# delehef/asgart

Measured on AMD Instinct MI355X. Metric: Mbp/s probe+extend (direct+RC, k=20 g=100), higher is better.
Workload: dtype u64 keys / u32 SA

## Files before the change

asgart_amd/__init__.py:

```python
from __future__ import annotations

import ctypes as C
import os
from dataclasses import dataclass, field
from typing import List, Optional, Sequence, Tuple

import numpy as np

__all__ = [
    "AsgartError", "RunSettings", "ProtoSD", "Strand", "Index", "Searcher", "SearchDuplications",
    "load_library", "library_path", "ABI_SYMBOLS", "sa_build64", "search_duplications_multi", "merge_shards",
    "score_owners", "score_costs", "compute_scores_multi", "Source", "compute_scores_flags_multi", "orientation_flags",
]

_HERE = os.path.dirname(os.path.abspath(__file__))

ABI_SYMBOLS = (
    "asgart_sa_build64", "asgart_index_create", "asgart_index_destroy", "asgart_index_prepare",
    "asgart_search_duplications", "asgart_search_duplications_shard", "asgart_families_counts",
    "asgart_families_copy", "asgart_families_free", "asgart_searcher_cache_get",
    "asgart_searcher_search", "asgart_sa_read", "asgart_probe_hits", "asgart_get_stats",
    "asgart_last_error", "asgart_version", "asgart_compute_scores", "asgart_index_set_option",
    "asgart_index_check_sa", "asgart_index_create_trim", "asgart_index_clone",
    "asgart_search_duplications_multi", "asgart_search_duplications_ex", "asgart_search_duplications_passes",
    "asgart_search_duplications_passes_shard", "asgart_families_keys",
    "asgart_index_export", "asgart_index_create_device", "asgart_trim_cache", "asgart_post_process",
    "asgart_debug_dump_stacks", "asgart_prepare_data", "asgart_score_owners", "asgart_score_costs",
    "asgart_compute_scores_shard", "asgart_compute_scores_multi", "asgart_tier_plan",
    "asgart_source_create", "asgart_source_destroy", "asgart_extract_sequences",
    "asgart_compute_scores_flags", "asgart_compute_scores_flags_shard", "asgart_compute_scores_flags_multi",
    "asgart_fasta_read", "asgart_fasta_counts", "asgart_fasta_copy", "asgart_fasta_read_text", "asgart_fasta_index",
    "asgart_fasta_source", "asgart_fasta_free", "asgart_fasta_timings", "asgart_fasta_geometry",
)


def merge_shards(parts) -> Tuple[np.ndarray, np.ndarray]:
    keys = np.concatenate([p[2] for p in parts]) if parts else np.zeros(0, np.uint64)
    if len(keys) == 0:
        return np.zeros(1, np.uint64), np.zeros((0, 4), np.uint64)
    starts = np.concatenate([p[0][:-1].astype(np.int64) + b for p, b in
                             zip(parts, np.cumsum([0] + [len(p[1]) for p in parts[:-1]]))])
    lens = np.concatenate([np.diff(p[0].astype(np.int64)) for p in parts])
    sds = np.concatenate([p[1] for p in parts])
    order = np.argsort(keys, kind="stable")
    lens_o, starts_o = lens[order], starts[order]
    offs = np.concatenate([[0], np.cumsum(lens_o)]).astype(np.uint64)
    idx = np.repeat(starts_o - offs[:-1].astype(np.int64), lens_o) + np.arange(int(offs[-1]), dtype=np.int64)
    return offs, sds[idx]


class AsgartError(RuntimeError):
    def __init__(self, code: int, msg: str):
        super().__init__(f"libasgart_hip error {code}: {msg}")
        self.code = code


def library_path() -> str:
    return os.environ.get("ASGART_LIB") or os.path.join(_HERE, "libasgart_hip.so")


class _Settings(C.Structure):
    _fields_ = [
        ("probe_size", C.c_uint64),
        ("max_gap_size", C.c_uint32),
        ("min_duplication_length", C.c_uint64),
        ("max_cardinality", C.c_uint64),
        ("reverse", C.c_uint8),
        ("complement", C.c_uint8),
    ]


class Stats(C.Structure):
    _fields_ = [("ms_total", C.c_double), ("ms_search", C.c_double), ("ms_scan", C.c_double),
                ("ms_fill", C.c_double), ("ms_extend", C.c_double)] + [
        (n, C.c_uint64) for n in (
            "probes_total", "probes_n_skipped", "probes_searched", "probes_card_skipped",
            "probes_with_hits", "raw_hits", "filtered_hits", "segments", "families", "proto_sds",
            "bisect_steps", "search_launches", "overflow_segments")] + [("ms_extend_tier2", C.c_double), ("heavy_segments", C.c_uint64), ("ms_probe_count", C.c_double),
        ("search_bytes", C.c_uint64), ("probes_filter_rejected", C.c_uint64), ("search_bytes_wide_loads", C.c_uint64),
        ("ms_longest_tier", C.c_double), ("passes", C.c_uint64), ("ms_longest_segment", C.c_double),
        ("split_segments", C.c_uint64), ("split_refused", C.c_uint64)]

    def as_dict(self):
        return {n: getattr(self, n) for n, _ in self._fields_}


_lib: Optional[C.CDLL] = None


def load_library() -> C.CDLL:
    global _lib
    if _lib is not None:
        return _lib
    path = library_path()
    if not os.path.exists(path):
        raise AsgartError(-3, f"{path} not built: run `python -c 'import __graft_entry__ as g; "
                              f"g.build()'` (hipcc --offload-arch=gfx950); there is no CPU fallback")
    L = C.CDLL(path)
    vp, u64p = C.c_void_p, C.POINTER(C.c_uint64)
    L.asgart_sa_build64.argtypes = [vp, vp, C.c_int64]
    L.asgart_sa_build64.restype = C.c_int32
    L.asgart_index_create.argtypes = [vp, C.c_int64, vp, C.c_int64, C.c_int32, C.POINTER(vp)]
    L.asgart_index_create.restype = C.c_int32
    L.asgart_index_create_trim.argtypes = [vp, C.c_int64, vp, C.c_int64, C.c_int64, C.c_int64, C.c_int32,
                                           C.POINTER(vp)]
    L.asgart_index_create_trim.restype = C.c_int32
    L.asgart_index_clone.argtypes = [vp, C.c_int32, C.POINTER(vp)]
    L.asgart_index_clone.restype = C.c_int32
    L.asgart_index_export.argtypes = [vp, C.POINTER(vp), C.POINTER(vp), C.POINTER(C.c_int32)]
    L.asgart_index_export.restype = C.c_int32
    L.asgart_index_create_device.argtypes = [vp, C.c_int64, vp, C.c_int64, C.c_int32, C.c_int32, C.POINTER(vp)]
    L.asgart_index_create_device.restype = C.c_int32
    L.asgart_trim_cache.argtypes = [C.c_int32]
    L.asgart_trim_cache.restype = C.c_int64
    L.asgart_prepare_data.argtypes = [vp, vp, C.c_int64, C.c_int32, C.c_int32, vp, vp, C.c_int64, C.POINTER(C.c_int64),
# ... 8 lines not shown
    L.asgart_fasta_read.argtypes = [vp, vp, C.c_int64, C.c_int32, C.c_int32, C.POINTER(vp)]
    L.asgart_fasta_read.restype = C.c_int32
    L.asgart_fasta_counts.argtypes = [vp, C.POINTER(C.c_int64), C.POINTER(C.c_int64), u64p]
    L.asgart_fasta_counts.restype = C.c_int32
    L.asgart_fasta_copy.argtypes = [vp, vp, vp, vp]
    L.asgart_fasta_copy.restype = C.c_int32
    L.asgart_fasta_read_text.argtypes = [vp, C.c_uint64, C.c_uint64, vp]
    L.asgart_fasta_read_text.restype = C.c_int32
    L.asgart_fasta_index.argtypes = [vp, C.POINTER(vp)]
    L.asgart_fasta_index.restype = C.c_int32
    L.asgart_fasta_source.argtypes = [vp, C.POINTER(vp)]
    L.asgart_fasta_source.restype = C.c_int32
    L.asgart_fasta_free.argtypes = [vp]
    L.asgart_fasta_free.restype = None
    L.asgart_fasta_timings.argtypes = [vp, C.POINTER(C.c_double)]
    L.asgart_fasta_timings.restype = C.c_int32
    L.asgart_fasta_geometry.argtypes = [u64p, u64p, u64p]
    L.asgart_fasta_geometry.restype = None
    L.asgart_debug_dump_stacks.argtypes = []
    L.asgart_debug_dump_stacks.restype = C.c_int32
    L.asgart_post_process.argtypes = [vp, vp, C.c_uint64, vp, C.c_int32, C.POINTER(vp)]
    L.asgart_post_process.restype = C.c_int32
    L.asgart_search_duplications_multi.argtypes = [C.POINTER(vp), C.c_int32, vp, C.c_int64, C.POINTER(_Settings), vp,
                                                   C.POINTER(vp)]
    L.asgart_search_duplications_multi.restype = C.c_int32
    L.asgart_index_destroy.argtypes = [vp]
    L.asgart_index_destroy.restype = None
    L.asgart_index_set_option.argtypes = [vp, C.c_char_p, C.c_int64]
    L.asgart_index_set_option.restype = C.c_int32
    L.asgart_index_check_sa.argtypes = [vp]
    L.asgart_index_check_sa.restype = C.c_int64
    L.asgart_index_prepare.argtypes = [vp, C.c_uint64]
    L.asgart_index_prepare.restype = C.c_int32
    L.asgart_search_duplications.argtypes = [vp, vp, C.c_int64, C.POINTER(_Settings), vp,
                                             C.POINTER(vp)]
    L.asgart_search_duplications.restype = C.c_int32
    L.asgart_search_duplications_shard.argtypes = [vp, vp, C.c_int64, C.POINTER(_Settings),
                                                   C.c_int32, C.c_int32, C.POINTER(vp)]
    L.asgart_search_duplications_shard.restype = C.c_int32
    L.asgart_search_duplications_ex.argtypes = [vp, vp, C.c_int64, C.POINTER(_Settings), C.c_int32, C.c_int32, vp,
                                                C.POINTER(vp)]
    L.asgart_search_duplications_ex.restype = C.c_int32
    L.asgart_search_duplications_passes.argtypes = [vp, vp, C.c_int64, C.POINTER(_Settings), C.c_int32, C.POINTER(vp)]
    L.asgart_search_duplications_passes.restype = C.c_int32
    L.asgart_families_keys.argtypes = [vp, vp]
    L.asgart_families_keys.restype = None
    L.asgart_search_duplications_passes_shard.argtypes = [vp, vp, C.c_int64, C.POINTER(_Settings), C.c_int32, C.c_int32,
                                                          C.c_int32, C.POINTER(vp)]
    L.asgart_search_duplications_passes_shard.restype = C.c_int32
    L.asgart_families_counts.argtypes = [vp, u64p, u64p]
    L.asgart_families_counts.restype = None
    L.asgart_families_copy.argtypes = [vp, vp, vp]
    L.asgart_families_copy.restype = None
    L.asgart_families_free.argtypes = [vp]
    L.asgart_families_free.restype = None
    L.asgart_searcher_cache_get.argtypes = [vp, vp, C.c_int64, vp, vp]
    L.asgart_searcher_cache_get.restype = C.c_int32
    L.asgart_searcher_search.argtypes = [vp, vp, C.c_int64, C.c_uint64, vp, vp]
    L.asgart_searcher_search.restype = C.c_int32
    L.asgart_sa_read.argtypes = [vp, C.c_uint64, C.c_uint64, vp]
    L.asgart_sa_read.restype = C.c_int32
    L.asgart_compute_scores.argtypes = [vp, vp, C.c_int64, C.c_int32, C.c_int32, vp]
    L.asgart_compute_scores.restype = C.c_int32
    L.asgart_score_owners.argtypes = [vp, C.c_int64, C.c_int32, vp]
    L.asgart_score_owners.restype = C.c_int32
    L.asgart_score_costs.argtypes = [vp, C.c_int64, vp]
    L.asgart_score_costs.restype = C.c_int32
    L.asgart_tier_plan.argtypes = [C.c_int32, vp, C.c_int64, vp, C.c_double, vp, vp]
    L.asgart_tier_plan.restype = C.c_int32
    L.asgart_compute_scores_shard.argtypes = [vp, vp, C.c_int64, C.c_int32, C.c_int32, C.c_int32, C.c_int32, vp]
    L.asgart_compute_scores_shard.restype = C.c_int64
    L.asgart_compute_scores_multi.argtypes = [C.POINTER(vp), C.c_int32, vp, C.c_int64, C.c_int32, C.c_int32, vp]
    L.asgart_compute_scores_multi.restype = C.c_int32
    L.asgart_compute_scores_flags.argtypes = [vp, vp, vp, C.c_int64, vp]
    L.asgart_compute_scores_flags.restype = C.c_int32
    L.asgart_compute_scores_flags_shard.argtypes = [vp, vp, vp, C.c_int64, C.c_int32, C.c_int32, vp]
    L.asgart_compute_scores_flags_shard.restype = C.c_int64
    L.asgart_compute_scores_flags_multi.argtypes = [C.POINTER(vp), C.c_int32, vp, vp, C.c_int64, vp]
    L.asgart_compute_scores_flags_multi.restype = C.c_int32
    L.asgart_probe_hits.argtypes = [vp, vp, C.c_int64, C.POINTER(_Settings), vp, vp, vp, u64p]
    L.asgart_probe_hits.restype = C.c_int64
    L.asgart_get_stats.argtypes = [vp, C.c_uint32, C.POINTER(Stats)]
    L.asgart_get_stats.restype = C.c_int32
    L.asgart_last_error.argtypes = []
    L.asgart_last_error.restype = C.c_char_p
    L.asgart_version.argtypes = []
    L.asgart_version.restype = C.c_char_p
    _lib = L
    return L


def _check(rc: int):
    if rc < 0:
        raise AsgartError(int(rc), load_library().asgart_last_error().decode(errors="replace"))


def _ptr(a: Optional[np.ndarray]):
    return None if a is None else a.ctypes.data_as(C.c_void_p)


def _as_u8(seq) -> np.ndarray:
    if isinstance(seq, np.ndarray):
        if seq.dtype != np.uint8:
            raise TypeError("text must be uint8")
        return np.ascontiguousarray(seq)
    if isinstance(seq, str):
        seq = seq.encode()
    return np.frombuffer(bytes(seq), dtype=np.uint8).copy()


@dataclass
class RunSettings:

    probe_size: int = 20
    max_gap_size: int = 120
    min_duplication_length: int = 1000
    max_cardinality: int = 500
    reverse: bool = False
    complement: bool = False
    skip_masked: bool = False
    trim: Optional[Tuple[int, int]] = None

    @classmethod
    def from_cli(cls, k=20, gap=100, min_length=1000, max_cardinality=500, reverse=False,
                 complement=False, skip_masked=False) -> "RunSettings":
        return cls(k, gap + k, min_length, max_cardinality, reverse, complement, skip_masked)

    def _c(self) -> _Settings:
        return _Settings(self.probe_size, self.max_gap_size, self.min_duplication_length,
                         self.max_cardinality, int(self.reverse), int(self.complement))


@dataclass
class ProtoSD:

    left: int
    right: int
    left_length: int
    right_length: int
    identity: float = 0.0
    reversed: bool = False
    complemented: bool = False

    def as_tuple(self):
        return (self.left, self.right, self.left_length, self.right_length)


ProtoSDsFamily = List[ProtoSD]


@dataclass
class Strand:

    file_names: str
    data: np.ndarray
    map: list = field(default_factory=list)


class Index:

    def __init__(self, text, sa: Optional[np.ndarray] = None, device: int = 0,
                 trim: Optional[Tuple[int, int]] = None):
        L = load_library()
        self.text = _as_u8(text)
        self.n = len(self.text)
        self._h = C.c_void_p()
        self.trim = trim
        sa_arr = None
        want = len(self.text) if trim is None else trim[1] - trim[0] + 1
        if sa is not None:
            sa_arr = np.ascontiguousarray(sa, dtype=np.int64)
            if len(sa_arr) != want:
                raise ValueError("suffix array length != text length (or the trimmed window + 1)")
        if trim is None:
            _check(L.asgart_index_create(_ptr(self.text), len(self.text), _ptr(sa_arr),
                                         want if sa_arr is not None else 0, device, C.byref(self._h)))
        else:
            _check(L.asgart_index_create_trim(_ptr(self.text), len(self.text), _ptr(sa_arr),
                                              want if sa_arr is not None else 0, int(trim[0]), int(trim[1]),
                                              device, C.byref(self._h)))

    def close(self):
        if getattr(self, "_h", None) and self._h.value:
            load_library().asgart_index_destroy(self._h)
            self._h = C.c_void_p()

    def __del__(self):
        try:
            self.close()
        except Exception:
            pass

    def __enter__(self):
        return self

    def __exit__(self, *exc):
        self.close()

    def clone(self, device: int = 0) -> "Index":
        other = Index.__new__(Index)
        other.text = self.text
        other.n = self.n
        other.trim = self.trim
        other._h = C.c_void_p()
        _check(load_library().asgart_index_clone(self._h, device, C.byref(other._h)))
        return other

    def export(self) -> Tuple[int, int, int]:
        t, a, w = C.c_void_p(), C.c_void_p(), C.c_int32()
        _check(load_library().asgart_index_export(self._h, C.byref(t), C.byref(a), C.byref(w)))
        return int(t.value), int(a.value), int(w.value)

    @classmethod
    def from_device(cls, d_text: int, n: int, d_sa: int, sa_entry_bytes: int, device: int = 0, text=None) -> "Index":
        self = cls.__new__(cls)
        self.text = text
        self.n = int(n)
        self.trim = None
        self._h = C.c_void_p()
        _check(load_library().asgart_index_create_device(C.c_void_p(d_text), n, C.c_void_p(d_sa), n, sa_entry_bytes,
                                                         device, C.byref(self._h)))
        return self

    def set_option(self, name: str, value: int):
        _check(load_library().asgart_index_set_option(self._h, name.encode(), int(value)))

    def check_sa(self) -> int:
        r = int(load_library().asgart_index_check_sa(self._h))
        _check(r)
        return r

    def prepare(self, probe_size: int):
        _check(load_library().asgart_index_prepare(self._h, probe_size))

    def sa_read(self, lo: int, hi: int) -> np.ndarray:
        out = np.empty(max(0, hi - lo), dtype=np.int64)
        _check(load_library().asgart_sa_read(self._h, lo, hi, _ptr(out)))
        return out

    def compute_scores(self, sds: np.ndarray, reversed_: bool = False, complemented: bool = False) -> np.ndarray:
        sds = np.ascontiguousarray(sds, dtype=np.uint64).reshape(-1, 4)
        out = np.empty(len(sds), dtype=np.float32)
        _check(load_library().asgart_compute_scores(self._h, _ptr(sds), len(sds), int(reversed_),
                                                    int(complemented), _ptr(out)))
        return out

    def compute_scores_shard(self, sds: np.ndarray, reversed_: bool = False, complemented: bool = False,
                             shard: int = 0, n_shards: int = 1) -> np.ndarray:
        sds = np.ascontiguousarray(sds, dtype=np.uint64).reshape(-1, 4)
        out = np.full(len(sds), np.nan, dtype=np.float32)
        _check(load_library().asgart_compute_scores_shard(self._h, _ptr(sds), len(sds), int(reversed_),
                                                          int(complemented), int(shard), int(n_shards), _ptr(out)))
        return out

    def compute_scores_flags(self, sds: np.ndarray, flags: Optional[np.ndarray]) -> np.ndarray:
        sds = np.ascontiguousarray(sds, dtype=np.uint64).reshape(-1, 4)
        flags = _score_flags(flags, len(sds))
        out = np.empty(len(sds), dtype=np.float32)
        _check(load_library().asgart_compute_scores_flags(self._h, _ptr(sds), _ptr(flags), len(sds), _ptr(out)))
        return out

    def compute_scores_flags_shard(self, sds: np.ndarray, flags: Optional[np.ndarray], shard: int = 0,
                                   n_shards: int = 1) -> np.ndarray:
        sds = np.ascontiguousarray(sds, dtype=np.uint64).reshape(-1, 4)
        flags = _score_flags(flags, len(sds))
        out = np.full(len(sds), np.nan, dtype=np.float32)
        _check(load_library().asgart_compute_scores_flags_shard(self._h, _ptr(sds), _ptr(flags), len(sds), int(shard),
                                                                int(n_shards), _ptr(out)))
        return out

    def post_process(self, offs: np.ndarray, sds: np.ndarray, threads: int = 0) -> Tuple[np.ndarray, np.ndarray]:
        L = load_library()
        offs = np.ascontiguousarray(offs, dtype=np.uint64)
        sds = np.ascontiguousarray(sds, dtype=np.uint64).reshape(-1, 4)
        h = C.c_void_p()
        _check(L.asgart_post_process(self._h, _ptr(offs), len(offs) - 1, _ptr(sds), threads, C.byref(h)))
        try:
            nf, ns = C.c_uint64(), C.c_uint64()
            L.asgart_families_counts(h, C.byref(nf), C.byref(ns))
            o = np.zeros(nf.value + 1, dtype=np.uint64)
            d = np.zeros((ns.value, 4), dtype=np.uint64)
            L.asgart_families_copy(h, _ptr(o), _ptr(d))
        finally:
            L.asgart_families_free(h)
        return o, d

    def stats(self, flags: int = 2) -> Stats:
        st = Stats()
        _check(load_library().asgart_get_stats(self._h, flags, C.byref(st)))
        return st

    def search_duplications_raw(self, chunks: Sequence[Tuple[int, int]], settings: RunSettings,
                                shard: int = 0, n_shards: int = 1, progress: Optional[np.ndarray] = None,
                                with_keys: bool = False):
        L = load_library()
        ch = np.array(chunks, dtype=np.uint64).reshape(-1)
        st = settings._c()
        h = C.c_void_p()
        if progress is not None:
            assert progress.dtype == np.uint64 and len(progress) >= len(chunks)
        if n_shards == 1:
            _check(L.asgart_search_duplications(self._h, _ptr(ch), len(chunks), C.byref(st), _ptr(progress),
                                                C.byref(h)))
        elif progress is None:
            _check(L.asgart_search_duplications_shard(self._h, _ptr(ch), len(chunks), C.byref(st),
                                                      shard, n_shards, C.byref(h)))
        else:
            _check(L.asgart_search_duplications_ex(self._h, _ptr(ch), len(chunks), C.byref(st), shard, n_shards,
# ... 94 lines not shown
        ends = np.zeros(2 * max(len(sds) - first, 1), dtype=np.uint64)
        done = C.c_int64()
        rc = load_library().asgart_extract_sequences(self._h, _ptr(sds), _ptr(flags), len(sds), int(first), _ptr(out),
                                                     len(out), _ptr(ends), C.byref(done))
        try:
            _check(rc)
        except AsgartError as err:
            if rc == -4:
                err.room = int(ends[1])
            raise
        return ends[:2 * done.value], int(done.value)

    def extract(self, sds: np.ndarray, reversed_=False, complemented=False,
                piece_bytes: int = 1 << 30) -> Tuple[np.ndarray, np.ndarray]:
        sds = np.ascontiguousarray(sds, dtype=np.uint64).reshape(-1, 4)
        n = len(sds)
        flags = (np.broadcast_to(np.asarray(reversed_, dtype=bool), (n,)).astype(np.uint8) |
                 (np.broadcast_to(np.asarray(complemented, dtype=bool), (n,)).astype(np.uint8) << 1))
        flags = np.ascontiguousarray(flags)
        total = int(sds[:, 2].sum(dtype=np.uint64) + sds[:, 3].sum(dtype=np.uint64)) if n else 0
        data = np.empty(total, dtype=np.uint8)
        ends = np.zeros(2 * n, dtype=np.uint64)
        first = pos = 0
        while first < n:
            cap = min(max(int(piece_bytes), 1), total - pos)
            try:
                e, done = self.extract_piece(sds, flags, first, data[pos:pos + cap])
            except AsgartError as err:
                if err.code != -4:
                    raise
                e, done = self.extract_piece(sds, flags, first, data[pos:pos + err.room])
            if done == 0:
                raise AsgartError(-4, f"asgart_extract_sequences: no progress at duplication {first}")
            ends[2 * first:2 * (first + done)] = e + np.uint64(pos)
            pos += int(e[-1]) if done else 0
            first += done
        return ends, data


def search_duplications_multi(indices: Sequence[Index], chunks: Sequence[Tuple[int, int]],
                              settings: RunSettings) -> Tuple[np.ndarray, np.ndarray]:
    L = load_library()
    ch = np.array(chunks, dtype=np.uint64).reshape(-1)
    st = settings._c()
    arr = (C.c_void_p * len(indices))(*[i._h for i in indices])
    h = C.c_void_p()
    _check(L.asgart_search_duplications_multi(arr, len(indices), _ptr(ch), len(chunks), C.byref(st), None,
                                              C.byref(h)))
    try:
        nf, ns = C.c_uint64(), C.c_uint64()
        L.asgart_families_counts(h, C.byref(nf), C.byref(ns))
        offs = np.zeros(nf.value + 1, dtype=np.uint64)
        sds = np.zeros((ns.value, 4), dtype=np.uint64)
        L.asgart_families_copy(h, _ptr(offs), _ptr(sds))
    finally:
        L.asgart_families_free(h)
    return offs, sds


def score_owners(sds: np.ndarray, n_shards: int) -> np.ndarray:
    sds = np.ascontiguousarray(sds, dtype=np.uint64).reshape(-1, 4)
    out = np.zeros(len(sds), dtype=np.int32)
    _check(load_library().asgart_score_owners(_ptr(sds), len(sds), int(n_shards), _ptr(out)))
    return out


def score_costs(sds: np.ndarray) -> np.ndarray:
    sds = np.ascontiguousarray(sds, dtype=np.uint64).reshape(-1, 4)
    out = np.zeros(len(sds), dtype=np.uint64)
    _check(load_library().asgart_score_costs(_ptr(sds), len(sds), _ptr(out)))
    return out


def tier_plan(budget: int, n_work, tier_order: int, est_ms, main_ms: float = 0.0) -> Tuple[np.ndarray, np.ndarray]:
    work = np.ascontiguousarray(n_work, dtype=np.uint64).reshape(7)
    est = np.ascontiguousarray(est_ms, dtype=np.float64).reshape(7)
    stream_of = np.zeros(7, dtype=np.int32)
    launch = np.zeros(7, dtype=np.int32)
    _check(load_library().asgart_tier_plan(int(budget), _ptr(work), int(tier_order), _ptr(est), float(main_ms),
                                           _ptr(stream_of), _ptr(launch)))
    return stream_of, launch


def compute_scores_multi(indices: Sequence[Index], sds: np.ndarray, reversed_: bool = False,
                         complemented: bool = False) -> np.ndarray:
    L = load_library()
    sds = np.ascontiguousarray(sds, dtype=np.uint64).reshape(-1, 4)
    out = np.empty(len(sds), dtype=np.float32)
    arr = (C.c_void_p * len(indices))(*[i._h for i in indices])
    _check(L.asgart_compute_scores_multi(arr, len(indices), _ptr(sds), len(sds), int(reversed_), int(complemented),
                                         _ptr(out)))
    return out


def _score_flags(flags, n: int) -> Optional[np.ndarray]:
    if flags is None:
        return None
    flags = np.ascontiguousarray(flags, dtype=np.uint8).reshape(-1)
    if len(flags) != n:
        raise ValueError(f"{len(flags)} flag bytes for {n} duplications")
    return flags


def orientation_flags(reversed_, complemented, n: Optional[int] = None) -> np.ndarray:
    f = np.asarray(reversed_, dtype=bool).astype(np.uint8) | (np.asarray(complemented, dtype=bool).astype(np.uint8) << 1)
    return np.ascontiguousarray(np.broadcast_to(f, (n,)) if n is not None else f)


def compute_scores_flags_multi(indices: Sequence[Index], sds: np.ndarray, flags: Optional[np.ndarray]) -> np.ndarray:
    sds = np.ascontiguousarray(sds, dtype=np.uint64).reshape(-1, 4)
    flags = _score_flags(flags, len(sds))
    out = np.empty(len(sds), dtype=np.float32)
    arr = (C.c_void_p * len(indices))(*[i._h for i in indices])
    _check(load_library().asgart_compute_scores_flags_multi(arr, len(indices), _ptr(sds), _ptr(flags), len(sds),
                                                            _ptr(out)))
    return out


def trim_cache(device: int = 0) -> int:
    r = int(load_library().asgart_trim_cache(device))
    _check(r)
    return r


def sa_build64(text) -> np.ndarray:
    t = _as_u8(text)
    sa = np.empty(len(t), dtype=np.int64)
    _check(load_library().asgart_sa_build64(_ptr(t), _ptr(sa), len(t)))
    return sa


class Searcher:

    def __init__(self, index: Index, offset: int = 0):
        self.index = index
        self.offset = offset

    @classmethod
    def new(cls, dna, sa: np.ndarray, offset: int = 0, device: int = 0) -> "Searcher":
        return cls(Index(dna, sa, device), offset)

    def cache(self, patterns8: Sequence[bytes]) -> List[Tuple[int, int]]:
        pats = np.frombuffer(b"".join(bytes(p) for p in patterns8), dtype=np.uint8).copy()
        n = len(patterns8)
        lo = np.zeros(n, dtype=np.uint64)
        hi = np.zeros(n, dtype=np.uint64)
        _check(load_library().asgart_searcher_cache_get(self.index._h, _ptr(pats), n, _ptr(lo),
                                                        _ptr(hi)))
        return [(int(a), int(b)) for a, b in zip(lo, hi)]

    def search_ranges(self, patterns: Sequence[bytes]) -> List[Tuple[int, int]]:
        k = len(patterns[0])
        pats = np.frombuffer(b"".join(bytes(p) for p in patterns), dtype=np.uint8).copy()
        n = len(patterns)
        lo = np.zeros(n, dtype=np.uint64)
        hi = np.zeros(n, dtype=np.uint64)
        _check(load_library().asgart_searcher_search(self.index._h, _ptr(pats), n, k, _ptr(lo),
                                                     _ptr(hi)))
        return [(int(a), int(b)) for a, b in zip(lo, hi)]

    def search(self, pattern: bytes) -> List[Tuple[int, int]]:
        (lo, hi), = self.search_ranges([pattern])
        starts = self.index.sa_read(lo, hi)
        k = len(pattern)
        return [(self.offset + int(x), self.offset + int(x) + k) for x in starts]

# ... 31 lines not shown
```

asgart_amd/csrc/device_base.hpp:

```cpp
#pragma once

#include "search_dev.hpp"

#include <type_traits>

namespace asgart {

constexpr int kTiers = 7;
constexpr int kRunsStat = kTiers + 1;

enum Counter {
    CT_BIG = 0,
    CT_SEG,
    CT_SCAN_TICKET,
    CT_FAM,
    CT_SD,
    CT_OVF,
    CT_TOTAL_HITS,
    CT_N_SKIPPED,
    CT_CARD_SKIPPED,
    CT_WITH_HITS,
    CT_RAW_HITS,
    CT_SEARCHED,
    CT_BISECT,
    CT_OVF_CURSOR,
    CT_AMBIG,
    CT_RANOUT,
    CT_EARLY_N = 34,
    CT_EARLY_CUR = 36,
    CT_RANK = 38,
    CT_BIG0 = 39,
    CT_ALG_BYTES = 68,
    CT_FLT_REJECTED,
    CT_LONGSEG,
    CT_ALG_BYTES16,
    CT_HIST_PEAK = 72,
    CT_HIST_PROBES = 88,
    CT_N1 = 104,
    CT_NF = 111,
    CT_CUR1 = 112,
    CT_CURF = 119,
    CT_OVF1 = 120,
    CT_BUSY1 = 128,
    CT_WGS1 = 136,
    CT_TPROBES1 = 144,
    CT_THITS1 = 152,
    CT_SEGMAX1 = 160,
    CT_CLUSTER_BARREN = 168,
    CT_CLUSTER_CUR = 169,
    CT_COUNT = 176
};

__device__ inline int chunk_of(const ChunkTable &ch, uint32_t g) {
    int lo = 0, hi = ch.n_chunks;
    while (hi - lo > 1) {
        int mid = (lo + hi) >> 1;
        if (ch.pbase[mid] <= g) lo = mid; else hi = mid;
    }
    return lo;
}

__device__ inline int chunk_of_uniform(const ChunkTable &ch, uint32_t g) {
    g = __builtin_amdgcn_readfirstlane(g);
    int lo = 0, hi = ch.n_chunks;
    while (hi - lo > 1) {
        const int mid = __builtin_amdgcn_readfirstlane((lo + hi) >> 1);
        if (ch.pbase[mid] <= g) lo = mid; else hi = mid;
    }
    return __builtin_amdgcn_readfirstlane(lo);
}

__device__ inline bool keep_hit(uint64_t x, uint64_t i, uint64_t s, uint64_t L, bool reverse) {
    if (!reverse) return x > i + s;
    return x != i && x >= s + L - i;
}

__device__ inline void lds_barrier() { __asm__ volatile("s_waitcnt lgkmcnt(0)\n\ts_barrier" ::: "memory"); }

__device__ inline uint32_t uni(uint32_t v) { return (uint32_t)__builtin_amdgcn_readfirstlane((int)v); }
__device__ inline unsigned long long uni(unsigned long long v) {
    return ((unsigned long long)uni((uint32_t)(v >> 32)) << 32) | uni((uint32_t)v);
}
__device__ inline uint32_t lane_of(uint32_t v, uint32_t l) {
    return (uint32_t)__builtin_amdgcn_readlane((int)v, (int)l);
}
__device__ inline unsigned long long lane_of(unsigned long long v, uint32_t l) {
    return ((unsigned long long)lane_of((uint32_t)(v >> 32), l) << 32) | lane_of((uint32_t)v, l);
}

__device__ inline uint32_t wave_incl_scan(uint32_t x) {
#define ASGART_DPP_ADD(ctrl, rows) \
    x += (uint32_t)__builtin_amdgcn_update_dpp(0, (int)x, ctrl, rows, 0xf, false)
    ASGART_DPP_ADD(0x111, 0xf);
    ASGART_DPP_ADD(0x112, 0xf);
    ASGART_DPP_ADD(0x114, 0xf);
    ASGART_DPP_ADD(0x118, 0xf);
    ASGART_DPP_ADD(0x142, 0xa);
    ASGART_DPP_ADD(0x143, 0xc);
#undef ASGART_DPP_ADD
    return x;
}

__device__ inline uint32_t wave_incl_max_scan(uint32_t x) {
#define ASGART_DPP_MAX(ctrl, rows) \
    x = max(x, (uint32_t)__builtin_amdgcn_update_dpp(0, (int)x, ctrl, rows, 0xf, false))
    ASGART_DPP_MAX(0x111, 0xf);
    ASGART_DPP_MAX(0x112, 0xf);
    ASGART_DPP_MAX(0x114, 0xf);
    ASGART_DPP_MAX(0x118, 0xf);
    ASGART_DPP_MAX(0x142, 0xa);
    ASGART_DPP_MAX(0x143, 0xc);
#undef ASGART_DPP_MAX
    return x;
}

}
```

asgart_amd/csrc/extend_common_dev.hpp:

```cpp
#pragma once

#include "device_base.hpp"

namespace asgart {

constexpr uint32_t kTombstone = 0xFFFFFFFFu;

#ifdef ASGART_PROFILE_EXTEND
#define PROF_DECL unsigned long long pf_t0 = 0, pf_acc[12] = {0, 0, 0, 0, 0, 0, 0, 0, 0, 0, 0, 0}
#define PROF_START() pf_t0 = __builtin_amdgcn_s_memtime()
#define PROF_STOP(slot) pf_acc[slot] += __builtin_amdgcn_s_memtime() - pf_t0
#define PROF_COUNT(slot, v) pf_acc[slot] += (v)
#define PROF_MAX(slot, v) pf_acc[slot] = pf_acc[slot] > (unsigned long long)(v) ? pf_acc[slot] : (unsigned long long)(v)
#define PROF_SEG_BEGIN() const unsigned long long pf_seg0 = __builtin_amdgcn_s_memtime()
#define PROF_FLUSH()                                                             \
    do {                                                                         \
        const unsigned long long pf_dt = __builtin_amdgcn_s_memtime() - pf_seg0; \
        if (lane == 0 && atomicMax(&P.ctr[28], pf_dt) < pf_dt) {                 \
            P.ctr[29] = g0;                                                      \
            P.ctr[30] = ((unsigned long long)pf_acc[5] << 32) | pf_acc[3];       \
            P.ctr[31] = ((unsigned long long)pf_acc[10] << 32) | pf_acc[11];     \
            P.ctr[32] = pf_acc[0];                                               \
            P.ctr[33] = pf_acc[6];                                               \
            P.ctr[25] = pf_acc[9];                                               \
// ... 25 lines not shown
#endif
constexpr int kHitBatch = 1024;
constexpr uint32_t kNoSeq = 0xFFFFFFFFu;

struct RangeRun {
    uint32_t g_begin, g_stop;
    uint32_t g_seg0;
    uint32_t emit_from;
    uint32_t flags;
    uint32_t split;
    uint32_t pad0, pad1;
};
constexpr uint32_t kRunNoEmit = 1u;
constexpr uint32_t kRunLast = 2u;
constexpr uint32_t kRunDumpCap = 5120;
template <class PosT> constexpr uint32_t kDumpWords = sizeof(PosT) == 4 ? 8u : 12u;
struct SplitSeg {
    uint32_t g_seg0, run_base, n_ranges, cut_base;
    uint32_t span, hits, tier, warm;
};

template <class PosT>
struct ExtParams {
    const RangeRun *runs;
    uint32_t *run_meta, *run_dump;
    RunParams rp;
    const uint32_t *p_filt;
    const unsigned long long *row_off;
    const PosT *hits;
    const uint32_t *seg_list;
    const unsigned long long *n_seg_ptr;
    unsigned long long *cursor;
    SdRec *recs;
    unsigned long long rec_cap;
    uint32_t *ovf_list;
    unsigned long long *ovf_count;
    char *scratch;
    uint32_t gen_bits;
    uint32_t escalate_cost;
    uint32_t cap_limit;
    uint32_t heavy_cap;
    uint32_t solo_hits;
    uint32_t k8_delay;
    uint32_t tier;
    unsigned long long *seg_slots;
    unsigned long long *ctr;
    unsigned long long *hb;
};

template <class PosT>
__device__ inline void heartbeat(const ExtParams<PosT> &P, uint32_t g0, uint32_t at) {
    if (P.hb) {
        unsigned long long *slot = P.hb + 2u * (blockIdx.x % 256u);
        __builtin_nontemporal_store((unsigned long long)g0 | 1ull << 63, slot);
        __builtin_nontemporal_store((unsigned long long)at, slot + 1);
    }
}

template <class PosT>
__device__ inline bool arm_accepts(PosT x, PosT re, uint32_t thr, uint32_t k) {
    const PosT lo = (PosT)(re - k + 1u);
    const uint64_t w = thr ? (uint64_t)thr + k - 1u : 0u;
    return (uint64_t)(PosT)(x - lo) < w;
}

__device__ inline uint32_t arm_threshold(uint64_t left_len, uint32_t G) {
    const uint64_t tenth = left_len <= 0xFFFFFFFFull ? (uint64_t)((uint32_t)left_len / 10u) : left_len / 10u;
    const uint64_t thr = tenth > (uint64_t)G ? tenth : (uint64_t)G;
    return thr > 0xFFFFFFFFull ? 0xFFFFFFFFu : (uint32_t)thr;
}

constexpr uint32_t kRecChunk = 32;
constexpr uint32_t kVoidStart = 0xFFFFFFFFu;
struct RecAlloc {
    unsigned long long next = 0;
    uint32_t left = 0;
};
template <class PosT>
__device__ inline void wg_begin(const ExtParams<PosT> &P) {
    if (threadIdx.x == 0 && P.tier >= 1u && P.tier <= (uint32_t)kRunsStat) {
        atomicAdd(&P.ctr[CT_BUSY1 + P.tier - 1u], 0ull - wall_clock64());
    }
}
template <class PosT>
__device__ inline void seg_clock(const ExtParams<PosT> &P, bool last = false) {
    if (!P.seg_slots || P.tier < 2u || P.tier > (uint32_t)kRunsStat) return;
    const unsigned long long now = wall_clock64();
    const unsigned long long prev = atomicExch(&P.seg_slots[blockIdx.x & 4095u], last ? 0ull : now);
    if (prev && now > prev) atomicMax(&P.ctr[CT_SEGMAX1 + P.tier - 1u], now - prev);
}
template <class PosT>
__device__ inline void wg_busy(const ExtParams<PosT> &P) {
    if (threadIdx.x == 0 && P.tier >= 1u && P.tier <= (uint32_t)kRunsStat) {
        seg_clock(P, true);
        atomicAdd(&P.ctr[CT_BUSY1 + P.tier - 1u], wall_clock64());
        atomicAdd(&P.ctr[CT_WGS1 + P.tier - 1u], 1ull);
    }
}
template <class PosT>
__device__ inline void rec_flush(RecAlloc &ra, const ExtParams<PosT> &P, int lane) {
    if ((uint32_t)lane < ra.left && ra.next + (unsigned)lane < P.rec_cap) P.recs[ra.next + (unsigned)lane].g_start = kVoidStart;
    ra.left = 0;
}
template <class PosT>
__device__ inline unsigned long long rec_slot(RecAlloc &ra, const ExtParams<PosT> &P, unsigned long long em, int lane) {
    const uint32_t n = (uint32_t)__popcll(em);
    if (n > ra.left) {
        rec_flush(ra, P, lane);
        const uint32_t take = n > kRecChunk ? n : kRecChunk;
        unsigned long long b = 0;
        if (lane == 0) b = atomicAdd(&P.ctr[CT_SD], (unsigned long long)take);
        ra.next = lane_of(b, 0u);
        ra.left = take;
    }
    const unsigned long long at = ra.next + (unsigned)__popcll(em & ((1ull << lane) - 1ull));
    ra.next += n;
    ra.left -= n;
    return at;
}

struct SegHeader {
    uint64_t cs, cl;
    bool rev;
    uint32_t pb;
    uint32_t chunk_end;
    uint32_t g_end;
};
__device__ inline SegHeader load_segment(const RunParams &rp, uint32_t g0) {
    const int c = chunk_of_uniform(rp.ch, g0);
    SegHeader s;
    s.cs = rp.ch.start[c];
    s.cl = rp.ch.len[c];
    s.rev = (rp.mode_of(c) & 2u) != 0u;
    s.pb = rp.ch.pbase[c];
    s.chunk_end = rp.ch.pbase[c + 1];
    s.g_end = min(s.chunk_end, rp.win_end(g0));
    return s;
}

struct ProbeBatch {
    uint32_t f_l, rel_l;
    unsigned long long base;
    uint32_t n;
    uint32_t tot;
    unsigned long long hm, qm;
};
template <int HB>
__device__ inline ProbeBatch load_batch(const uint32_t *p_filt, const unsigned long long *row_off, uint32_t g, uint32_t g_end,
                                        int lane) {
    ProbeBatch b;
    const uint32_t nb = min(64u, g_end - g);
    b.f_l = (uint32_t)lane < nb ? p_filt[g + lane] : kSkipN;
    const unsigned long long r_l = (uint32_t)lane < nb ? row_off[g + lane] : 0ull;
    const unsigned long long r_hi = uni(row_off[g + nb]);
    b.base = lane_of(r_l, 0u);
    unsigned long long r_next = __shfl_down(r_l, 1);
    if ((uint32_t)lane + 1 >= nb) r_next = r_hi;
    const bool fits = (uint32_t)lane < nb && r_next - b.base <= (unsigned long long)HB;
    const unsigned long long fm = __ballot(fits);
    b.n = (~fm == 0ull) ? 64u : (uint32_t)(__ffsll((long long)~fm) - 1);
    if (b.n > nb) b.n = nb;
    b.rel_l = (uint32_t)(r_l - b.base);
    b.tot = (uint32_t)((b.n == nb ? r_hi : lane_of(r_l, b.n)) - b.base);
    const unsigned long long in_batch = b.n >= 64 ? ~0ull : ((1ull << b.n) - 1ull);
    b.hm = __ballot(b.f_l >= 1u && b.f_l < kPending) & in_batch;
    b.qm = __ballot(b.f_l == 0u) & in_batch;
    return b;
}
__device__ inline uint32_t next_hit(const ProbeBatch &b, uint32_t pos, uint32_t &quiet_before) {
    const unsigned long long hmr = pos >= 64 ? 0ull : (b.hm >> pos) << pos;
    const uint32_t at = hmr ? (uint32_t)(__ffsll((long long)hmr) - 1) : 64u;
    const unsigned long long upto = at >= 64 ? ~0ull : ((1ull << at) - 1ull);
// ... 48 lines not shown
```

asgart_amd/csrc/index.hip:

```cpp
#include "index.hpp"
#include "search_dev.hpp"

#include <algorithm>
#include <cctype>
#include <cerrno>
#include <chrono>
#include <cstdlib>

#include <dirent.h>
#include <execinfo.h>
#include <signal.h>
#include <sys/syscall.h>
#include <unistd.h>

namespace asgart {

static thread_local char g_err[512] = "";
thread_local bool tl_owns_pass_mu = false;

void set_error(const char *fmt, ...) {
    va_list ap;
    va_start(ap, fmt);
    vsnprintf(g_err, sizeof(g_err), fmt, ap);
    va_end(ap);
// ... 1051 lines not shown
                if (idx->wide)
                    add_offset_kernel<uint64_t><<<grid_capped((uint64_t)n_sa), 256, 0, s>>>((uint64_t *)idx->d_sa, (uint64_t)n_sa, (uint64_t)trim_start);
                else
                    add_offset_kernel<uint32_t><<<grid_capped((uint64_t)n_sa), 256, 0, s>>>((uint32_t *)idx->d_sa, (uint64_t)n_sa, (uint64_t)trim_start);
                HIP_TRY(hipGetLastError());
                HIP_TRY(stream_sync(s));
                return 0;
            }();
            sub.release();
            RC_TRY(rc2);
        } else if (!SA) {
            RC_TRY(sa_build_device(idx->d_text, n, idx->d_sa, idx->wide, idx->ctx[0].stream,
                                   (uint64_t)idx->opt.test_wide_batch));
        } else if (idx->wide) {
            HIP_TRY(hipMemcpyAsync(idx->d_sa, SA, (size_t)n_sa * 8, hipMemcpyHostToDevice,
                                   idx->ctx[0].stream));
            HIP_TRY(stream_sync(idx->ctx[0].stream));
        } else {
            const uint64_t slice = 1ull << 25;
            DevBuf stage;
            RC_TRY(stage.reserve((size_t)(slice < (uint64_t)n_sa ? slice : (uint64_t)n_sa) * 8));
            for (uint64_t off = 0; off < (uint64_t)n_sa; off += slice) {
                uint64_t cnt = (uint64_t)n_sa - off < slice ? (uint64_t)n_sa - off : slice;
                hipError_t e = hipMemcpyAsync(stage.p, SA + off, cnt * 8, hipMemcpyHostToDevice,
                                              idx->ctx[0].stream);
                if (e == hipSuccess) {
                    narrow_sa_kernel<<<grid_for(cnt), 256, 0, idx->ctx[0].stream>>>(
                        stage.as<int64_t>(), (uint32_t *)idx->d_sa + off, cnt);
                    e = hipStreamSynchronize(idx->ctx[0].stream);
                }
                if (e != hipSuccess) {
                    stage.release();
                    HIP_TRY(e);
                }
            }
            stage.release();
        }
        return 0;
    }();
    if (rc != 0) {
        asgart_index_destroy(idx);
        return rc;
    }
    *out = idx;
    return 0;
}

int32_t asgart_index_create(const uint8_t *T, int64_t n, const int64_t *SA, int64_t sa_len,
                            int32_t device, asgart_index **out) {
    return index_create_impl(T, n, SA, sa_len, false, 0, 0, device, out);
}

int32_t asgart_index_create_trim(const uint8_t *T, int64_t n, const int64_t *SA, int64_t sa_len,
                                 int64_t trim_start, int64_t trim_end, int32_t device,
                                 asgart_index **out) {
    return index_create_impl(T, n, SA, sa_len, true, trim_start, trim_end, device, out);
}

int32_t asgart_index_clone(asgart_index *src, int32_t device, asgart_index **out) {
    if (!out) {
        set_error("asgart_index_clone: out is NULL");
        return ASGART_E_ARG;
    }
    *out = nullptr;
    if (!src) {
        set_error("asgart_index_clone: source index is NULL");
        return ASGART_E_ARG;
    }
    RC_TRY(check_device(device));
    asgart_index *idx = new (std::nothrow) asgart_index();
    if (!idx) {
        set_error("out of host memory");
        return ASGART_E_OOM;
    }
    BlockCache::index_born();
    idx->device = device;
    idx->n = src->n;
    idx->n_sa = src->n_sa;
    idx->trimmed = src->trimmed;
    idx->trim_start = src->trim_start;
    idx->trim_end = src->trim_end;
    idx->wide = src->wide;
    idx->opt = src->opt;
    idx->h_tail = src->h_tail;
    for (auto &cx : idx->ctx) memset(&cx.stats, 0, sizeof(cx.stats));
    src->acquire_all();
    int32_t rc = [&]() -> int32_t {
        HIP_TRY(hipSetDevice(device));
        for (auto &cx : idx->ctx) RC_TRY(create_ctx_streams(cx));
        const size_t slot = idx->wide ? 8 : 4;
        const size_t text_bytes = (size_t)idx->n + 64, sa_bytes = ((size_t)idx->n_sa + 16) * slot;
        HIP_TRY(dev_malloc((void **)&idx->d_text, text_bytes));
        HIP_TRY(dev_malloc(&idx->d_sa, sa_bytes));
        hipStream_t s = idx->ctx[0].stream;
        HIP_TRY(hipMemcpyPeerAsync(idx->d_text, device, src->d_text, src->device, text_bytes, s));
        HIP_TRY(hipMemcpyPeerAsync(idx->d_sa, device, src->d_sa, src->device, sa_bytes, s));
        HIP_TRY(stream_sync(s));
        return 0;
    }();
    src->release_all();
    if (rc != 0) {
        asgart_index_destroy(idx);
        return rc;
    }
    *out = idx;
    return 0;
}

int64_t asgart_trim_cache(int32_t device) {
    RC_TRY(check_device(device));
    (void)bounded_call(60.0, []() {});
    const size_t held = BlockCache::held();
    BlockCache::trim();
    return (int64_t)held;
}

int32_t asgart_index_export(asgart_index *idx, const void **d_text, const void **d_sa, int32_t *sa_entry_bytes) {
    if (!idx) {
        set_error("index is NULL");
        return ASGART_E_ARG;
    }
    if (d_text) *d_text = idx->d_text;
    if (d_sa) *d_sa = idx->d_sa;
    if (sa_entry_bytes) *sa_entry_bytes = idx->wide ? 8 : 4;
    return 0;
}

int32_t asgart_index_create_device(const void *d_text, int64_t n, const void *d_sa, int64_t sa_len,
                                   int32_t sa_entry_bytes, int32_t device, asgart_index **out) {
    if (!out) {
        set_error("asgart_index_create_device: out is NULL");
        return ASGART_E_ARG;
    }
    *out = nullptr;
    if (!d_text || n <= 0 || sa_len != n) {
        set_error("asgart_index_create_device: need the text (and a suffix array of the same length, or NULL) on the device");
        return ASGART_E_ARG;
    }
    RC_TRY(check_device(device));
    asgart::Options opt;
    options_from_env(opt);
    const bool wide = (uint64_t)n >= 0xFFFFFF00ull || opt.force_wide != 0;
    if (sa_entry_bytes != (wide ? 8 : 4)) {
        set_error("asgart_index_create_device: a text of %lld bytes takes %d-byte suffix-array entries here (got %d)",
                  (long long)n, wide ? 8 : 4, sa_entry_bytes);
        return ASGART_E_ARG;
    }
    asgart_index *idx = new (std::nothrow) asgart_index();
    if (!idx) {
        set_error("out of host memory");
        return ASGART_E_OOM;
    }
    BlockCache::index_born();
    idx->device = device;
    idx->n = n;
    idx->n_sa = n;
    idx->opt = opt;
    idx->wide = wide;
    for (auto &cx : idx->ctx) memset(&cx.stats, 0, sizeof(cx.stats));
    int32_t rc = [&]() -> int32_t {
        for (auto &cx : idx->ctx) RC_TRY(create_ctx_streams(cx));
        hipStream_t s = idx->ctx[0].stream;
        const size_t slot = wide ? 8 : 4;
        HIP_TRY(dev_malloc((void **)&idx->d_text, (size_t)n + 64));
        HIP_TRY(dev_malloc(&idx->d_sa, ((size_t)n + 16) * slot));
        prealloc_ptab(idx);
        HIP_TRY(hipMemsetAsync(idx->d_text + n, 0, 64, s));
        HIP_TRY(hipMemcpyAsync(idx->d_text, d_text, (size_t)n, hipMemcpyDeviceToDevice, s));
        if (d_sa) HIP_TRY(hipMemcpyAsync(idx->d_sa, d_sa, (size_t)n * slot, hipMemcpyDeviceToDevice, s));
        bool dna = false;
        RC_TRY(text_is_dna(idx->d_text, n, s, &dna));
        if (!d_sa && dna)
            RC_TRY(sa_build_device(idx->d_text, n, idx->d_sa, idx->wide, s, (uint64_t)idx->opt.test_wide_batch));
        const int64_t tl = n < (int64_t)kMaxK + 32 ? n : (int64_t)kMaxK + 32;
        idx->h_tail.resize((size_t)tl);
        HIP_TRY(read_back(idx->h_tail.data(), idx->d_text + (n - tl), (size_t)tl, s));
        HIP_TRY(stream_sync(s));
        if (!dna) {
            set_error("text contains bytes other than the normalised bases {A,C,G,T,N} and '$' "
                      "(reference src/bin/asgart.rs:289-301,430)");
            return ASGART_E_ARG;
        }
        return 0;
    }();
    if (rc != 0) {
        asgart_index_destroy(idx);
        return rc;
    }
    *out = idx;
    return 0;
}

int32_t asgart_index_set_option(asgart_index *idx, const char *name, int64_t value) {
    if (!idx) {
        set_error("index is NULL");
        return ASGART_E_ARG;
    }
    if (name && (!strcmp(name, "force_wide") || !strcmp(name, "ptab_depth"))) {
        set_error("option %s is fixed when the index is created (set ASGART_<NAME> in the environment before)", name);
        return ASGART_E_ARG;
    }
    idx->acquire_all();
    const int32_t rc = option_set(idx->opt, name, value);
    if (rc == 0 && !strcmp(name, "test_fail_alloc")) asgart::fail_alloc_countdown().store(value);
    idx->release_all();
    return rc;
}

int64_t asgart_index_check_sa(asgart_index *idx) {
    if (!idx) {
        set_error("index is NULL");
        return ASGART_E_ARG;
    }
    if (idx->trimmed) {
        set_error("asgart_index_check_sa: not for a --trim index (its array covers a window of the text)");
        return ASGART_E_ARG;
    }
    REFUSE_POISONED(idx);
    HIP_TRY(hipSetDevice(idx->device));
    idx->acquire_all();
    struct Unlock {
        asgart_index *i;
        ~Unlock() { i->release_all(); }
    } unlock{idx};
    const uint64_t n = (uint64_t)idx->n;
    const size_t slot = idx->wide ? 8 : 4;
    DevBuf isa, errs;
    hipStream_t s = idx->ctx[0].stream;
    unsigned long long h_errs = 0;
    int32_t rc = [&]() -> int32_t {
        RC_TRY(isa.reserve(n * slot));
        RC_TRY(errs.reserve(8));
        HIP_TRY(hipMemsetAsync(isa.p, 0xFF, n * slot, s));
        HIP_TRY(hipMemsetAsync(errs.p, 0, 8, s));
        const unsigned g = grid_capped(n);
        if (idx->wide) {
            isa_scatter_kernel<uint64_t><<<g, 256, 0, s>>>((const uint64_t *)idx->d_sa, isa.as<uint64_t>(), n);
            sa_check_kernel<uint64_t><<<g, 256, 0, s>>>(idx->d_text, (const uint64_t *)idx->d_sa, isa.as<uint64_t>(), n,
                                                        errs.as<unsigned long long>());
        } else {
            isa_scatter_kernel<uint32_t><<<g, 256, 0, s>>>((const uint32_t *)idx->d_sa, isa.as<uint32_t>(), n);
            sa_check_kernel<uint32_t><<<g, 256, 0, s>>>(idx->d_text, (const uint32_t *)idx->d_sa, isa.as<uint32_t>(), n,
                                                        errs.as<unsigned long long>());
        }
        HIP_TRY(hipGetLastError());
        HIP_TRY(read_back(&h_errs, errs.p, 8, s));
        HIP_TRY(stream_sync(s));
        return 0;
    }();
    isa.release();
    errs.release();
    if (rc != 0) return rc;
    return (int64_t)h_errs;
}

int32_t asgart_index_prepare(asgart_index *idx, uint64_t probe_size) {
    if (!idx) {
        set_error("index is NULL");
        return ASGART_E_ARG;
    }
    return index_prepare(idx, probe_size);
}

static bool pattern_bytes_ok(const uint8_t *p, int64_t cnt) {
    for (int64_t j = 0; j < cnt; ++j) {
        uint8_t c = p[j];
        if (!(c == 'A' || c == 'C' || c == 'G' || c == 'T' || c == 'N')) return false;
    }
    return true;
}

static int32_t run_pattern_kernel(asgart_index *idx, const uint8_t *pats, int64_t n_pat,
                                  int64_t width, bool cache, uint64_t *lo, uint64_t *hi) {
    if (n_pat == 0) return 0;
    REFUSE_POISONED(idx);
    HIP_TRY(hipSetDevice(idx->device));
    idx->acquire_all();
    struct Unlock {
        asgart_index *i;
        ~Unlock() { i->release_all(); }
    } unlock{idx};
    Workspace &w = idx->ctx[0].ws;
    RC_TRY(w.pat.reserve((size_t)(n_pat * width)));
    RC_TRY(w.out_a.reserve((size_t)n_pat * 8));
    RC_TRY(w.out_b.reserve((size_t)n_pat * 8));
    hipStream_t s = idx->ctx[0].stream;
    HIP_TRY(hipMemcpyAsync(w.pat.p, pats, (size_t)(n_pat * width), hipMemcpyHostToDevice, s));
    unsigned g = grid_for((uint64_t)n_pat);
    if (idx->wide) {
// ... 87 lines not shown
```

asgart_amd/csrc/index.hpp:

```cpp
#pragma once

#include "common.hpp"

#include <functional>
#include <memory>
#include <thread>
#include <condition_variable>
#include <mutex>

namespace asgart {

template <class SlotT>
struct IndexView {
    const uint8_t *text;
    const SlotT *sa;
    const uint64_t *keys;
    const SlotT *ptab;
    const SlotT *c8lo;
    const SlotT *c8hi;
    uint64_t n;
    int k;
    int kk;
    int k2;
    int d;
// ... 50 lines not shown
    __host__ __device__ inline uint32_t tiles_per_window(uint32_t tile) const { return (win_len + tile - 1u) / tile; }
    __host__ __device__ inline uint32_t n_tiles(uint32_t tile) const { return n_passes * tiles_per_window(tile); }
    __host__ __device__ inline uint32_t tile_of(uint32_t t, uint32_t tile, uint32_t &end) const {
        const uint32_t tw = tiles_per_window(tile);
        const uint32_t w = n_passes <= 1u ? 0u : (t >= tw ? 1u : 0u) + (t >= 2u * tw ? 1u : 0u) + (t >= 3u * tw ? 1u : 0u);
        const uint32_t lo = win_lo(w);
        end = lo + win_len;
        return lo + (t - w * tw) * tile;
    }
};

struct SdRec {
    uint32_t g_start;
    uint32_t fam_seq;
    uint32_t create_seq;
    uint32_t pad;
    asgart_proto_sd sd;
};

struct Workspace {
    DevBuf chunks;
    DevBuf p_lo;
    DevBuf p_raw;
    DevBuf p_filt;
    DevBuf row_off;
    DevBuf blk;
    DevBuf hits;
    DevBuf big_list;
    DevBuf rank_list;
    DevBuf seg_list;
    DevBuf counters;
    DevBuf fam_sds;
    DevBuf ovf_list;
    DevBuf scratch;
    DevBuf seg_keys, seg_vals, sort_tmp;
    DevBuf rec_k32, rec_k64, rec_idx, rec_sorted;
    DevBuf pat;
    DevBuf out_a, out_b;
    DevBuf seg_info;
    DevBuf seg_slots;
    DevBuf split_buf;
    DevBuf split_dump;
    void release_all() {
        DevBuf *bufs[] = {&chunks, &p_lo, &p_raw, &p_filt, &row_off, &blk, &hits, &big_list, &rank_list, &seg_list,
                          &counters, &fam_sds, &ovf_list, &scratch, &seg_keys, &seg_vals,
                          &sort_tmp, &rec_k32, &rec_k64, &rec_idx, &rec_sorted, &pat, &out_a, &out_b, &seg_info, &seg_slots, &split_buf, &split_dump};
        static_assert(sizeof(Workspace) == sizeof(bufs) / sizeof(bufs[0]) * sizeof(DevBuf),
                      "a buffer of the workspace is missing from release_all");
        for (DevBuf *b : bufs) b->release();
    }
};

}

namespace asgart {
enum CtxEvent {
    EV_SEARCH,
    EV_PROBE_COUNT,
    EV_SEARCHED,
    EV_SCANNED,
    EV_FILL,
    EV_HIT_ROWS,
    EV_BARREN,
    EV_BARREN_SMALL,
    EV_BARREN_BIG,
    EV_TIERS,
    EV_EXTENDED,
    EV_COUNT
};
struct SearchCtx {
    static constexpr int kMaxTierStreams = 6;
    hipStream_t stream = nullptr;
    hipStream_t tier_st[kMaxTierStreams] = {};
    int n_tier_st = 0;
    hipStream_t fill_stream = nullptr;
    hipEvent_t ev[EV_COUNT] = {};
    hipEvent_t tier_ev[7] = {};
    hipEvent_t runs_ev = nullptr;
    uint64_t plan_sig = 0;
    bool plan_known = false;
    double plan_est[8] = {};
    Workspace ws;
    asgart_stats stats;
    RunParams last_rp;
    bool has_last = false;
    bool raw_done = false;
    uint32_t last_P = 0;
    bool busy = false;
    volatile uint64_t *progress = nullptr;
    void *h_pinned = nullptr;
    size_t h_pinned_cap = 0;
    struct FamPart {
        std::vector<asgart_proto_sd> sds[4];
        std::vector<uint64_t> ends[4], keys[4];
    };
    std::vector<FamPart> fam_parts;
    int32_t pinned(size_t bytes, void **out) {
        if (bytes > h_pinned_cap) {
            if (h_pinned) (void)hipHostFree(h_pinned);
            h_pinned = nullptr;
            h_pinned_cap = 0;
            const size_t want = bytes + bytes / 4 + 4096;
            if (hipHostMalloc(&h_pinned, want, hipHostMallocDefault) != hipSuccess) {
                (void)hipGetLastError();
                h_pinned = nullptr;
                set_error("hipHostMalloc(%zu bytes) failed", want);
                return ASGART_E_OOM;
            }
            h_pinned_cap = want;
        }
        *out = h_pinned;
        return 0;
    }
    static constexpr int kHbTiers = 8, kHbSlots = 256;
    unsigned long long *h_hb = nullptr;
    unsigned long long *d_hb = nullptr;
    int32_t heartbeat(bool want) {
        if (!want || h_hb) return 0;
        void *hp = nullptr, *dp = nullptr;
        if (hipHostMalloc(&hp, (size_t)kHbTiers * kHbSlots * 16, hipHostMallocMapped) != hipSuccess ||
            hipHostGetDevicePointer(&dp, hp, 0) != hipSuccess) {
            (void)hipGetLastError();
            if (hp) (void)hipHostFree(hp);
            return 0;
        }
        memset(hp, 0, (size_t)kHbTiers * kHbSlots * 16);
        h_hb = static_cast<unsigned long long *>(hp);
        d_hb = static_cast<unsigned long long *>(dp);
        return 0;
    }
    void *h_ctl = nullptr;
    size_t h_ctl_cap = 0;
    int32_t ctl(size_t bytes, void **out) {
        if (bytes > h_ctl_cap) {
            if (h_ctl) (void)hipHostFree(h_ctl);
            h_ctl = nullptr;
            h_ctl_cap = 0;
            const size_t want = bytes + 65536;
            if (hipHostMalloc(&h_ctl, want, hipHostMallocDefault) != hipSuccess) {
                (void)hipGetLastError();
                h_ctl = nullptr;
                set_error("hipHostMalloc(%zu bytes) failed", want);
                return ASGART_E_OOM;
            }
            h_ctl_cap = want;
        }
        *out = h_ctl;
        return 0;
    }
};
constexpr int kNumCtx = 2;

struct Options {
    int64_t shard_lookback = 4096;
    int64_t shard_lookahead = 0;
    int64_t force_tier = 0;
    int64_t arms_kernel = 1;
    int64_t long3 = 16384;
    int64_t cap1 = 256;
    int64_t debug = 0;
    int64_t test_cap_limit = -1;
    int64_t test_genbits = 22;
    int64_t test_k8_delay = 0;
    int64_t tier_order = 3654217;
    int64_t grid[8] = {0, 0, 0, 0, 0, 0, 0, 0};
    int64_t ptab_depth = 0;
    int64_t force_wide = 0;
    int64_t test_wide_batch = 0;
    int64_t rank_lists = 1;
    int64_t cap6_pct = 140;
    int64_t test_fail_alloc = -1;
    int64_t solo = 1;
    int64_t cap6w_pct = 160;
    int64_t cap45_pct = 100;
    int64_t cap3_pct = 160;
    int64_t posbits = 1;
    int64_t barren = 2;
    int64_t fuse_passes = 1;
    int64_t fuse_pole_pct = 88;
    int64_t lazy_aux = 1;
    int64_t dense3 = 16;
    int64_t dense6 = 32;
    int64_t split = 1;
    int64_t split_len = 0;
    int64_t split_runs = 224;
    int64_t split_warm = 6144;
    int64_t split_warm_max = 65536;
    int64_t split_min = 0;
    int64_t cache_calls = 2;
    int64_t prewarm = 1;
    int64_t test_stall_s = 0;
    int64_t watchdog_s = 120;
};
int32_t create_ctx_streams(SearchCtx &cx);
int hw_queue_budget();
int32_t tier_plan(int budget, const uint64_t *n_work, int64_t tier_order, const double *est_ms, double main_ms,
                  int32_t *stream_of, int32_t *launch);
template <class SlotT>
int32_t build_rank_lists_runs(const uint64_t *d_keys, const SlotT *d_sa, uint64_t n, SlotT *d_sap, uint32_t min_run, int k,
                              hipStream_t s);
int32_t option_set(Options &o, const char *name, int64_t value);
void options_from_env(Options &o);
}

namespace asgart {
struct PassWorker {
    std::mutex m;
    std::condition_variable cv;
    std::function<void()> job;
    bool busy = false, stop = false;
    std::thread th;
    PassWorker() : th([this] { loop(); }) {}
    ~PassWorker() {
        {
            std::lock_guard<std::mutex> lk(m);
            stop = true;
        }
        cv.notify_all();
        th.join();
    }
    void loop() {
        std::unique_lock<std::mutex> lk(m);
        for (;;) {
            cv.wait(lk, [&] { return stop || (busy && job); });
            if (stop) return;
            std::function<void()> j = std::move(job);
            job = nullptr;
            lk.unlock();
            j();
            lk.lock();
            busy = false;
            cv.notify_all();
        }
    }
    void submit(std::function<void()> j) {
        {
            std::lock_guard<std::mutex> lk(m);
            job = std::move(j);
            busy = true;
        }
        cv.notify_all();
    }
    void wait() {
        std::unique_lock<std::mutex> lk(m);
        cv.wait(lk, [&] { return !busy; });
    }
};
}

struct asgart_index {
    int device = 0;
    int64_t n = 0;
    int64_t n_sa = 0;
    bool trimmed = false;
    int64_t trim_start = 0, trim_end = 0;
    int n_bad = 0;
    uint64_t bad[asgart::kMaxK + 2] = {};
    bool wide = false;
    uint8_t *d_text = nullptr;
    void *d_sa = nullptr;
    uint64_t k = 0;
    int d = 0;
    uint64_t *d_keys = nullptr;
    void *d_ptab = nullptr;
    uint64_t ptab_entries = 0;
    void *d_c8lo = nullptr;
    void *d_c8hi = nullptr;
    void *d_sap = nullptr;
    uint64_t *d_pbits[4] = {nullptr, nullptr, nullptr, nullptr};
    bool filter_off[4] = {false, false, false, false};
    uint64_t pbits_uses[4] = {0, 0, 0, 0};
    uint32_t tail8[asgart::kMaxK];
    int n_tail8 = 0;
    uint64_t tail_bloom = 0;
    std::vector<uint8_t> h_tail;
    bool sap_tried = false;
    uint64_t calls_total = 0;
    double ms_prepare = 0.0;
    std::atomic<bool> poisoned{false};
    double tail_ms[4] = {-1.0, -1.0, -1.0, -1.0};
    asgart::Options opt;
    asgart::SearchCtx ctx[asgart::kNumCtx];
    int last_ctx = 0;
    std::mutex mu;
    std::condition_variable cv;
    struct FuseVerdict {
        uint64_t k = 0, M = 0, C = 0, modes = 0;
        uint32_t G = 0;
        int32_t n_passes = 0, shard = 0, n_shards = 1;
        bool seen = false, pole = false;
        int32_t n_fused = 0, n_piped = 0;
        int32_t unsettled = 0;
        double ms_fused = 1e30, ms_piped = 1e30;
    } fuse_verdict;
    struct SplitVerdict {
        uint64_t key, sig;
        uint32_t allowed, range_len;
        uint32_t warm;
    };
    std::vector<SplitVerdict> split_blocked;
    asgart::DevBuf ws_arena;
    std::mutex pass_mu;
    std::vector<std::unique_ptr<asgart::PassWorker>> pass_workers;

    asgart::SearchCtx &acquire_one(int *which) {
        std::unique_lock<std::mutex> lk(mu);
        for (;;) {
            for (int i = 0; i < asgart::kNumCtx; ++i)
                if (!ctx[i].busy) {
                    ctx[i].busy = true;
                    *which = i;
                    return ctx[i];
                }
            cv.wait(lk);
        }
    }
    void acquire_all() {
        std::unique_lock<std::mutex> lk(mu);
        for (;;) {
            bool any = false;
            for (auto &c : ctx) any |= c.busy;
            if (!any) break;
            cv.wait(lk);
        }
        for (auto &c : ctx) c.busy = true;
    }
    void release_one(int which) {
        {
            std::lock_guard<std::mutex> lk(mu);
            ctx[which].busy = false;
            last_ctx = which;
        }
        cv.notify_all();
    }
    void release_all() {
        {
            std::lock_guard<std::mutex> lk(mu);
            for (auto &c : ctx) c.busy = false;
        }
        cv.notify_all();
    }

    template <class SlotT>
    asgart::IndexView<SlotT> view() const {
        asgart::IndexView<SlotT> v;
        v.text = d_text;
        v.sa = reinterpret_cast<const SlotT *>(d_sa);
        v.keys = d_keys;
        v.ptab = reinterpret_cast<const SlotT *>(d_ptab);
        v.c8lo = reinterpret_cast<const SlotT *>(d_c8lo);
        v.c8hi = reinterpret_cast<const SlotT *>(d_c8hi);
        v.n = (uint64_t)n;
        v.k = (int)k;
        v.kk = (int)std::min<uint64_t>(k, (uint64_t)asgart::kMaxKey);
        v.k2 = v.k - v.kk;
        v.d = d;
        for (int j = 0; j < asgart::kMaxK; ++j) v.tail8[j] = tail8[j];
        v.n_tail8 = n_tail8;
        v.tail_bloom = tail_bloom;
        v.sap = reinterpret_cast<const SlotT *>(d_sap);
        v.n_sa = (uint64_t)n_sa;
        v.trim = trimmed ? 1 : 0;
        v.n_bad = n_bad;
        for (int j = 0; j < asgart::kMaxK + 2; ++j) v.bad[j] = bad[j];
// ... 43 lines not shown
```

asgart_amd/csrc/pipeline.hip:

```cpp
#include "pipeline_dev.hpp"
#include "extend_wave_dev.hpp"
#include "extend_heavy_dev.hpp"
#include "extend_fast_dev.hpp"
#include "extend_k8_dev.hpp"

#include <algorithm>
#include <atomic>
#include <chrono>
#include <string>
#include <thread>
#include <utility>

namespace asgart {

#ifdef ASGART_PROFILE_EXTEND
#define PROF_DUMP(tag)                                                                          \
    do {                                                                                       \
        fprintf(stderr, "[extend profile %s] stage=%llu batches=%llu | reg_cyc=%llu reg_probes=%llu | build=%llu "\
                "lds_probes=%llu match=%llu apply=%llu retire=%llu segs=%llu sumA=%llu sumCnt=%llu | longest: "   \
                "cyc=%llu g0=%llu lds_probes=%llu reg_probes=%llu sumA=%llu sumCnt=%llu stage=%llu match=%llu\n", \
                tag, h_ctr[16], h_ctr[17], h_ctr[18], h_ctr[19], h_ctr[20], h_ctr[21], h_ctr[22], h_ctr[23],  \
                h_ctr[24], h_ctr[25], h_ctr[26], h_ctr[27], h_ctr[28], h_ctr[29], h_ctr[30] >> 32,            \
                h_ctr[30] & 0xffffffffull, h_ctr[31] >> 32, h_ctr[31] & 0xffffffffull, h_ctr[32], h_ctr[33]); \
        fprintf(stderr, "    K7 steps=%llu; cycles [to barrier 1, wait, to barrier 2, wait]: control %llu %llu %llu %llu | arm wave 0 %llu %llu %llu %llu | last arm wave %llu %llu %llu %llu\n", \
                h_ctr[52], h_ctr[40], h_ctr[41], h_ctr[42], h_ctr[43], h_ctr[44], h_ctr[45], h_ctr[46], h_ctr[47], h_ctr[48], h_ctr[49], h_ctr[50], h_ctr[51]); \
        fprintf(stderr, "    K7 wave 0: extra row rounds %llu, stash rounds %llu, arms offered cooperatively %llu, resolved cooperatively %llu\n", h_ctr[53], h_ctr[56], h_ctr[54], h_ctr[55]); \
        fprintf(stderr, "    K7 wave 0 cycles: A[cmd %llu resolve %llu offers %llu] B[mid %llu create+offers %llu publish %llu next-cmd+index %llu]\n", h_ctr[57], h_ctr[58], h_ctr[59], h_ctr[60], h_ctr[61], h_ctr[62], h_ctr[63]); \
        (void)hipMemsetAsync(d_ctr + 52, 0, 13 * 8, s);                                        \
        fprintf(stderr, "    P1: arm lookups=%llu linear=%llu chain nodes=%llu accepts=%llu by level:", h_ctr[40], h_ctr[41], h_ctr[42], h_ctr[43]); \
        for (int pf_i = 0; pf_i < 8; ++pf_i) fprintf(stderr, " %llu", h_ctr[44 + pf_i]);       \
        fprintf(stderr, "\n");                                                                 \
        (void)hipMemsetAsync(d_ctr + 40, 0, 12 * 8, s);                                        \
        fprintf(stderr, "    longest slots:");                                                  \
        for (int pf_i = 0; pf_i < 12; ++pf_i) fprintf(stderr, " [%d]=%llu", pf_i, h_ctr[56 + pf_i]); \
        fprintf(stderr, "\n");                                                                 \
        fprintf(stderr, "    segments by peak arms (log2 bins):");                             \
        for (int pf_i = 0; pf_i < 16; ++pf_i) fprintf(stderr, " %llu", h_ctr[CT_HIST_PEAK + pf_i]); \
        fprintf(stderr, "\n    probes by segment length (log2 bins):");                        \
        for (int pf_i = 0; pf_i < 16; ++pf_i) fprintf(stderr, " %llu", h_ctr[CT_HIST_PROBES + pf_i]); \
        fprintf(stderr, "\n");                                                                 \
        (void)hipMemsetAsync(d_ctr + 16, 0, 18 * 8, s);                                        \
        (void)hipMemsetAsync(d_ctr + 56, 0, (CT_N1 - 56) * 8, s);                              \
    } while (0)
#define PROF_TIER(tag, stream, n)                                                               \
    do {                                                                                       \
        const auto pf_c0 = std::chrono::steady_clock::now();                                   \
        (void)hipStreamSynchronize(stream);                                                    \
        const double pf_ms = std::chrono::duration<double, std::milli>(std::chrono::steady_clock::now() - pf_c0).count(); \
        (void)hipMemcpy(h_ctr, d_ctr, kCtrBytes, hipMemcpyDeviceToHost);                   \
        fprintf(stderr, "[tier %s] segments=%llu  %.2f ms\n", tag, (unsigned long long)(n), pf_ms); \
        PROF_DUMP(tag);                                                                        \
        (void)hipStreamSynchronize(s);                                                         \
    } while (0)
#else
#define PROF_DUMP(tag)
#define PROF_TIER(tag, stream, n)
#endif

enum class TierKernel {
    none,
    wave,
    fast,
    k8,
    heavy_lds,
    heavy_hybrid,
    heavy_hbm
};
static_assert((int)TierKernel::heavy_hybrid == (int)TierKernel::heavy_lds + 1 && (int)TierKernel::heavy_hbm == (int)TierKernel::heavy_lds + 2,
              "extend_heavy_kernel's MODE is the distance from heavy_lds");
struct TierShape {
    TierKernel kernel;
    int threads;
    int layers, slots;
    int hits, rows;
    int wg_per_cu;
    int grid;
    int64_t Options::*widen;
    bool early;
    double profile_ms;
    constexpr uint32_t cap() const { return (uint32_t)(layers * slots); }
};
template <class SlotT>
struct TierTable {
    static constexpr bool k32 = sizeof(SlotT) == 4;
    static constexpr int kLong = k32 ? 2048 : 1024;
    static constexpr TierShape kNone = {TierKernel::none, 0, 0, 0, 0, 0, 1, 0, nullptr, false, 0.0};
    static constexpr TierShape kWave = {TierKernel::wave, 64, 1, 256, kHitBatch, 0, 11, 256 * 8, nullptr, false, 4.6};
    static constexpr TierShape kHbm = {TierKernel::heavy_hbm, kHeavyThreads, 1, 1, kHitBatch, 0, 1, 256, nullptr, false, 33.0};
    static constexpr TierShape kK8 = {TierKernel::k8, 1024, k32 ? 5 : 4, 896, kHitBatch, kLong, 1, 256, &Options::cap3_pct, true, 67.0};
    static constexpr TierShape shape[kTiers + 1][2] = {
        {{kK8.kernel, kK8.threads, kK8.layers, kK8.slots, kK8.hits, kK8.rows, 1, 0, nullptr, false, 67.0}, kNone},
        {kWave, kWave},
        {{TierKernel::fast, 64, k32 ? 8 : 5, 64, 512, 256, 8, 256 * 8, nullptr, false, 51.8},
         {TierKernel::heavy_lds, kMidThreads, 1, 768, kHitBatch, 0, 3, 256 * 3, nullptr, false, 51.8}},
        {kK8, kNone},
        {{TierKernel::fast, 256, k32 ? 4 : 2, 256, 512, 512, 4, 256 * 4, &Options::cap45_pct, false, 35.5},
         {TierKernel::heavy_lds, kHeavyThreads, 1, k32 ? 2432 : 1664, kHitBatch, 0, 1, 256, nullptr, false, 35.5}},
        {{TierKernel::fast, 512, k32 ? 4 : 2, 512, kHitBatch, 1024, 2, 256 * 2, &Options::cap45_pct, false, 53.0}, kNone},
        {{TierKernel::fast, 1024, k32 ? 5 : 4, 1024, kHitBatch, kLong, 1, 256, k32 ? &Options::cap6_pct : &Options::cap6w_pct, true, 33.0},
         {TierKernel::heavy_hybrid, kHeavyThreads, 1, k32 ? 4608 : 3072, kHitBatch, 0, 1, 256, nullptr, true, 33.0}},
        {kHbm, kHbm},
    };
    static constexpr int kRunsTier = 3;
};
template <class SlotT>
constexpr bool tier_caps(int set, uint32_t c1, uint32_t c2, uint32_t c3, uint32_t c4, uint32_t c5, uint32_t c6) {
    const uint32_t want[kTiers] = {0, c1, c2, c3, c4, c5, c6};
    for (int t = 1; t < kTiers; ++t)
        if (TierTable<SlotT>::shape[t][set].cap() != want[t]) return false;
    return true;
}
static_assert(tier_caps<uint32_t>(0, 256, 512, 4480, 1024, 2048, 5120) && tier_caps<uint64_t>(0, 256, 320, 3584, 512, 1024, 4096),
              "capacities of the arm-resident set");
static_assert(tier_caps<uint32_t>(1, 256, 768, 0, 2432, 0, 4608) && tier_caps<uint64_t>(1, 256, 768, 0, 1664, 0, 3072),
              "capacities of the LDS-array set");
constexpr uint32_t kTier1MaxSum = 20000;

static inline unsigned grid_for(uint64_t n, unsigned block = 256) {
    return (unsigned)((n + block - 1) / block);
}

__global__ void stall_kernel(unsigned long long ticks) {
    const unsigned long long t0 = wall_clock64();
    while (wall_clock64() - t0 < ticks) __builtin_amdgcn_s_sleep(100);
}

static uint32_t probes_in_chunk(uint64_t L, uint64_t k, uint64_t step, uint64_t M) {
    if (L < M || L < k + step || L - k - step == 0) return 0;
    return (uint32_t)((L - k - step + step - 1) / step);
}

struct Watchdog {
    asgart_index *idx;
    SearchCtx &cx;
    std::chrono::steady_clock::time_point t0, t_change;
    unsigned long long sig = 0;
    Watchdog(asgart_index *i, SearchCtx &c) : idx(i), cx(c), t0(std::chrono::steady_clock::now()), t_change(t0) {}
    unsigned long long signature() const {
        unsigned long long h = 1469598103934665603ull;
        if (cx.h_hb) {
            const volatile unsigned long long *p = cx.h_hb;
            for (int i = 0; i < SearchCtx::kHbTiers * SearchCtx::kHbSlots * 2; ++i) h = (h ^ p[i]) * 1099511628211ull;
        }
        return h;
    }
    bool expired(const char *phase) {
        const int64_t limit_s = idx->opt.watchdog_s;
        if (limit_s <= 0) return false;
        const auto now = std::chrono::steady_clock::now();
        const unsigned long long s2 = signature();
        if (s2 != sig) {
            sig = s2;
            t_change = now;
        }
        if (std::chrono::duration<double>(now - t_change).count() <= (double)limit_s) return false;
        std::string who;
        if (cx.h_hb) {
            int shown = 0;
            for (int t = 0; t < SearchCtx::kHbTiers && shown < 12; ++t)
                for (int w = 0; w < SearchCtx::kHbSlots && shown < 12; ++w) {
                    const unsigned long long a = cx.h_hb[2 * (t * SearchCtx::kHbSlots + w)], b = cx.h_hb[2 * (t * SearchCtx::kHbSlots + w) + 1];
                    if (!(a >> 63)) continue;
                    char buf[96];
                    snprintf(buf, sizeof buf, "%s tier %d wg %d: segment at probe %llu, position %llu", shown ? ";" : "", t, w,
                             a & 0xFFFFFFFFull, b);
                    who += buf;
                    ++shown;
                }
        }
        idx->poisoned.store(true);
        set_error("watchdog: no progress for %lld s while waiting for %s (%.1f s into the wait); last heartbeats:%s -- the index is "
                  "unusable from here on (option watchdog_s = 0 waits forever)", (long long)limit_s, phase,
                  std::chrono::duration<double>(now - t0).count(), who.empty() ? " none" : who.c_str());
        return true;
    }
};

static int32_t wd_sync(asgart_index *idx, SearchCtx &cx, hipStream_t st, const char *phase) {
    if (idx->opt.watchdog_s <= 0) {
        HIP_TRY(hipStreamSynchronize(st));
        return 0;
    }
    Watchdog wd(idx, cx);
// ... 13 lines not shown
        return 0;
    }
    Watchdog wd(idx, cx);
    for (unsigned spins = 0;; ++spins) {
        const hipError_t q = hipEventQuery(ev);
        if (q == hipSuccess) return 0;
        if (q != hipErrorNotReady) HIP_TRY(q);
        (void)hipGetLastError();
        if (spins < 64) continue;
        std::this_thread::sleep_for(std::chrono::microseconds(spins < 2000 ? 20 : 500));
        if ((spins & 1023u) == 0 && wd.expired(phase)) return ASGART_E_HIP;
    }
}

int32_t reserve_probe_workspace(asgart_index *idx, SearchCtx &cx, uint64_t W) {
    Workspace &w = cx.ws;
    const uint64_t n_blk = (W + kScanTile - 1) / kScanTile + 4;
    RC_TRY(w.p_lo.reserve((size_t)W * (idx->wide ? 8 : 4)));
    RC_TRY(w.p_raw.reserve((size_t)W * 4));
    RC_TRY(w.p_filt.reserve((size_t)W * 4));
    RC_TRY(w.row_off.reserve(((size_t)W + 1) * 8));
    RC_TRY(w.blk.reserve((size_t)n_blk * sizeof(ScanEl)));
    RC_TRY(w.big_list.reserve((size_t)W * 4));
    if (idx->d_sap) RC_TRY(w.rank_list.reserve((size_t)W * 4));
    RC_TRY(w.counters.reserve(CT_COUNT * 8));
    return 0;
}

bool carve_probe_workspace(asgart_index *idx, const uint64_t *Wc) {
    if (idx->ws_arena.p) return false;
    size_t off = 0;
    struct Piece {
        DevBuf *b;
        size_t off, bytes;
    };
    std::vector<Piece> pieces;
    for (int c = 0; c < kNumCtx; ++c) {
        Workspace &w = idx->ctx[c].ws;
        const uint64_t W = Wc[c];
        const uint64_t n_blk = (W + kScanTile - 1) / kScanTile + 4;
        DevBuf *bufs[7] = {&w.p_lo, &w.p_raw, &w.p_filt, &w.row_off, &w.blk, &w.big_list, &w.rank_list};
        const size_t want[7] = {(size_t)W * (idx->wide ? 8 : 4), (size_t)W * 4, (size_t)W * 4, ((size_t)W + 1) * 8,
                                (size_t)n_blk * sizeof(ScanEl), (size_t)W * 4, (size_t)W * 4};
        for (int j = 0; j < 7; ++j) {
            if (bufs[j]->p) return false;
            const size_t sz = (want[j] + 4095) & ~(size_t)4095;
            pieces.push_back(Piece{bufs[j], off, sz});
            off += sz;
        }
    }
    size_t cap = 0;
    void *p = BlockCache::take(off, &cap, 30);
    if (!p) return false;
    idx->ws_arena.p = p;
    idx->ws_arena.cap = cap;
    for (const Piece &pc : pieces) {
        pc.b->p = static_cast<char *>(p) + pc.off;
        pc.b->cap = pc.bytes;
        pc.b->view = true;
    }
    return true;
}

template <class SlotT>
struct SearchCall {

    asgart_index *const idx;
    SearchCtx &cx;
    const uint64_t *const chunks;
    const int64_t n_chunks_pass;
    const asgart_settings *const sts;
    const int32_t n_passes, shard, n_shards;
    const bool want_csr;
    asgart_families *const *const fams;
    std::vector<uint8_t> *const status_out;
    std::vector<uint64_t> *const rowoff_out, *const hits_out;
    Workspace &w;
    const hipStream_t s;
    const asgart_settings *const st;
    const bool fam_out;
    const int64_t n_chunks;
    const uint64_t k, step, n;
    const Options opt;
    static constexpr size_t kCtrBytes = (size_t)CT_COUNT * 8;
    static constexpr size_t kSplitMirror = 512 << 10;
    using Tiers = TierTable<SlotT>;
    static constexpr int caph = (int)Tiers::shape[6][1].cap();
    bool nothing_to_do = true;
    size_t ch_bytes = 0;
    unsigned long long *h_ctr = nullptr, *h_scalar = nullptr;
    uint64_t *h_start = nullptr, *h_len = nullptr;
    uint32_t *h_pbase = nullptr;
    char *h_split = nullptr;
    std::vector<uint32_t> lp;
    uint32_t Ppass = 0, P = 0, own_lo = 0, own_hi = 0, lo_lim = 0, hi_lim = 0, K = 0;
    uint64_t look_back = 0, look_ahead = 0, call_sig = 0;
    uint64_t *d_start = nullptr, *d_len = nullptr;
    uint32_t *d_pbase = nullptr;
    std::chrono::steady_clock::time_point t_host0, t_launch;
    RunParams rp;
    uint32_t W = 0, W_probes = 0;
    unsigned long long *d_ctr = nullptr;
    IndexView<SlotT> ix;
    SlotT *p_lo = nullptr, *hits = nullptr;
    uint32_t *p_raw = nullptr, *p_filt = nullptr, *seg_list = nullptr;
    unsigned long long *row_off = nullptr;
    uint64_t total_hits = 0, n_seg = 0, n_overflow = 0, n_heavy = 0;
    bool progress_given = false;
    uint64_t rec_cap = 0;
    const SdRec *h_recs = nullptr;
    size_t n_hrec = 0;
    bool arms_kernel = false, split_on = false;
    uint32_t tier_cap[kTiers + 1] = {};
    char *d_split = nullptr;
    const uint32_t *order = nullptr;
    uint64_t n_t[kTiers] = {}, seg_off[kTiers + 1] = {};
    uint64_t h_tp[kTiers] = {}, h_th[kTiers] = {};
    const unsigned long long *h_split_hdr = nullptr;
    uint32_t n_runs = 0, n_cuts = 0, n_splits = 0;
    std::vector<SplitSeg> split_segs;
    uint32_t *ovf[kTiers] = {};
    uint64_t heavy_cap64 = 0;
    unsigned n_wg7 = 1;
    size_t region = 0;
    char *scratch6 = nullptr, *scratch7 = nullptr;
    ExtParams<SlotT> base{};
    hipStream_t tier_stream[kTiers + 1] = {};
    bool tier_ran[kTiers + 1] = {};
    uint64_t early_n[kTiers + 1] = {};
    double ms_tier2 = 0.0, ms_longest_tier = 0.0, ms_longest_segment = 0.0;
    uint64_t n_split_segments = 0, n_split_refused = 0;

    SearchCall(asgart_index *idx_, SearchCtx &cx_, const uint64_t *chunks_, int64_t n_chunks_pass_, const asgart_settings *sts_,
               int32_t n_passes_, int32_t shard_, int32_t n_shards_, bool want_csr_, asgart_families *const *fams_,
               std::vector<uint8_t> *status_out_, std::vector<uint64_t> *rowoff_out_, std::vector<uint64_t> *hits_out_)
        : idx(idx_), cx(cx_), chunks(chunks_), n_chunks_pass(n_chunks_pass_), sts(sts_), n_passes(n_passes_), shard(shard_),
          n_shards(n_shards_), want_csr(want_csr_), fams(fams_), status_out(status_out_), rowoff_out(rowoff_out_),
          hits_out(hits_out_), w(cx_.ws), s(cx_.stream), st(&sts_[0]), fam_out(fams_ != nullptr),
          n_chunks(n_chunks_pass_ * (int64_t)n_passes_), k(sts_[0].probe_size), step(sts_[0].probe_size / 2),
          n((uint64_t)idx_->n), opt(idx_->opt) {}

    uint32_t pass_of_probe(uint32_t g) const { return std::min<uint32_t>(g / K, (uint32_t)n_passes - 1u); }
    uint32_t pass_offset(uint32_t g) const { return lo_lim + (g - pass_of_probe(g) * K); }
    const TierShape &shape(int t) const { return Tiers::shape[t][arms_kernel ? 0 : 1]; }
    bool tier_enabled(int t) const { return t >= 1 && t <= kTiers && tier_cap[t] != 0; }
    int next_holding_more(int src) const {
        int dst = src + 1;
        while (dst < kTiers && (!tier_enabled(dst) || tier_cap[dst] <= tier_cap[src])) ++dst;
        return dst;
    }
    double since_launch() const {
        return std::chrono::duration<double, std::milli>(std::chrono::steady_clock::now() - t_launch).count();
    }
    void signal_progress() {
        for (int64_t c = 0; c < n_chunks_pass; ++c)
            cx.progress[c] = (uint64_t)probes_in_chunk(h_len[c], k, step, st->min_duplication_length) * step;
        progress_given = true;
    }

    static constexpr uint32_t kMaxRuns = 4096, kMaxCuts = 2048, kMaxSplits = 1024;
    static constexpr size_t kOffRuns = 64, kOffCuts = kOffRuns + kMaxRuns * sizeof(RangeRun), kOffSplits = kOffCuts + kMaxCuts * 8,
                     kOffMeta = kOffSplits + kMaxSplits * sizeof(SplitSeg), kOffOk = kOffMeta + kMaxRuns * 64,
                     kOffFix = kOffOk + kMaxCuts * 4, kOffAgain = kOffFix + kMaxRuns * 4, kOffChoice = kOffAgain + kMaxSplits * 4,
                     kOffBlocked = kOffChoice + 128, kSplitBytes = kOffBlocked + kSplitBlockedMax * sizeof(BlockedSeg);
    static_assert(sizeof(SplitChoice) <= 128 && kOffChoice % 8 == 0, "split choice");
    static_assert(kSplitBytes <= kSplitMirror, "split mirror");

    int32_t setup() {
        ch_bytes = (size_t)n_chunks * 16 + ((size_t)n_chunks + 1) * 4;
        void *ctl_p = nullptr;
        RC_TRY(cx.ctl(kCtrBytes + ch_bytes + 256 + 64 + kSplitMirror, &ctl_p));
        h_ctr = static_cast<unsigned long long *>(ctl_p);
        h_scalar = h_ctr + CT_COUNT;
        h_start = reinterpret_cast<uint64_t *>(static_cast<char *>(ctl_p) + kCtrBytes + 256);
        h_len = h_start + n_chunks;
        h_pbase = reinterpret_cast<uint32_t *>(h_len + n_chunks);
        h_split = reinterpret_cast<char *>((reinterpret_cast<uintptr_t>(h_pbase + n_chunks + 1) + 63u) & ~(uintptr_t)63u);
        const uint64_t text_end = (idx->h_tail.size() && idx->h_tail.back() == '$') ? n - 1 : n;
        lp.assign((size_t)n_chunks_pass + 1, 0u);
        {
            uint64_t P64 = 0;
            for (int64_t c = 0; c < n_chunks_pass; ++c) {
                const uint64_t c_start = chunks[2 * c], c_len = chunks[2 * c + 1];
                if (c_start > text_end || c_len > text_end - c_start) {
                    set_error("chunk %lld = (%llu, %llu) exceeds the text (%llu bases before '$')",
                              (long long)c, (unsigned long long)c_start, (unsigned long long)c_len, (unsigned long long)text_end);
                    return ASGART_E_ARG;
                }
                lp[(size_t)c] = (uint32_t)P64;
                P64 += probes_in_chunk(c_len, k, step, st->min_duplication_length);
                if (P64 * (uint64_t)n_passes >= 0xFFFFFF00ull) {
                    set_error("more than 2^32 probes in one call");
                    return ASGART_E_CAP;
                }
            }
            lp[(size_t)n_chunks_pass] = (uint32_t)P64;
        }
        Ppass = lp[(size_t)n_chunks_pass];
        P = Ppass * (uint32_t)n_passes;
        cx.last_P = P;
        memset(&cx.stats, 0, sizeof(cx.stats));
        cx.stats.probes_total = P;
        if (fam_out)
            for (int32_t p = 0; p < n_passes; ++p) {
                fams[p]->fam_offsets.assign(1, 0);
                fams[p]->fam_keys.clear();
                fams[p]->sds.clear();
            }
        if (want_csr) {
            status_out->assign(P, 0);
            rowoff_out->assign((size_t)P + 1, 0);
            hits_out->clear();
        }
        if (P == 0 || n_chunks == 0) return 0;
        if (want_csr && (n_shards != 1 || n_passes != 1)) {
            set_error("asgart_probe_hits is one unsharded pass");
            return ASGART_E_ARG;
        }
        own_lo = (uint32_t)((uint64_t)Ppass * (uint64_t)shard / (uint64_t)n_shards);
        own_hi = (uint32_t)((uint64_t)Ppass * (uint64_t)(shard + 1) / (uint64_t)n_shards);
        if (own_lo == own_hi) return 0;
        look_back = (uint64_t)opt.shard_lookback;
        look_ahead = opt.shard_lookahead > 0 ? (uint64_t)opt.shard_lookahead
                                                      : std::max<uint64_t>(65536, (own_hi - own_lo) / 16);
        const int64_t c0 = (int64_t)(std::upper_bound(lp.begin(), lp.end(), own_lo) - lp.begin()) - 1;
        const int64_t c1 = (int64_t)(std::upper_bound(lp.begin(), lp.end(), own_hi - 1u) - lp.begin()) - 1;
        lo_lim = lp[(size_t)c0];
        hi_lim = lp[(size_t)c1 + 1];
        K = hi_lim - lo_lim;
        for (int64_t c = 0; c < n_chunks; ++c) {
            const int64_t cl = c % n_chunks_pass, p = c / n_chunks_pass;
            h_start[c] = chunks[2 * cl];
            h_len[c] = chunks[2 * cl + 1];
// ... 108 lines not shown
        HIP_TRY(hipEventRecord(cx.ev[EV_FILL], sf));
        fill_small_kernel<SlotT><<<rp.n_tiles(256u), 256, 0, sf>>>(ix, rp, p_lo, p_raw, p_filt, row_off, hits);
        if (h_ctr[CT_BIG])
            fill_big_kernel<SlotT><<<2048, 256, 0, sf>>>(ix, rp, p_lo, p_raw, p_filt, row_off, hits,
                                                         big_list, d_ctr);
        HIP_TRY(hipEventRecord(cx.ev[EV_HIT_ROWS], sf));
        HIP_TRY(hipGetLastError());

        return 0;
    }

    int32_t csr_out() {
        std::vector<uint32_t> h_filt(P);
        std::vector<SlotT> h_hits((size_t)total_hits);
        RC_TRY(wd_sync(idx, cx, s, "the hit rows"));
        HIP_TRY(hipMemcpyAsync(h_filt.data(), p_filt, (size_t)P * 4, hipMemcpyDeviceToHost, s));
        HIP_TRY(hipMemcpyAsync(rowoff_out->data(), row_off, ((size_t)P + 1) * 8,
                               hipMemcpyDeviceToHost, s));
        if (total_hits)
            HIP_TRY(hipMemcpyAsync(h_hits.data(), hits, (size_t)total_hits * sizeof(SlotT),
                                   hipMemcpyDeviceToHost, s));
        HIP_TRY(hipStreamSynchronize(s));
        for (uint32_t g = 0; g < P; ++g)
            (*status_out)[g] = h_filt[g] == kSkipN ? 1 : (h_filt[g] == kSkipCard ? 2 : 0);
        hits_out->resize((size_t)total_hits);
        for (uint64_t j = 0; j < total_hits; ++j) (*hits_out)[j] = h_hits[j];
        return 0;
    }

    int32_t place() {
        rec_cap = std::max<uint64_t>(1u << 18, w.fam_sds.cap / sizeof(SdRec));
        RC_TRY(w.ovf_list.reserve((size_t)(n_seg + 1) * 4 * kTiers));
        h_recs = nullptr;
        n_hrec = 0;
        const int force_tier = (int)opt.force_tier;
        RC_TRY(w.seg_keys.reserve((size_t)n_seg * 4 * 2));
        RC_TRY(w.seg_vals.reserve((size_t)n_seg * 4 * 2));
        uint32_t *kbuf = w.seg_keys.as<uint32_t>(), *vbuf = w.seg_vals.as<uint32_t>();
        HIP_TRY(hipMemsetAsync(d_ctr + CT_N1, 0, (size_t)(CT_COUNT - CT_N1) * 8, s));
        arms_kernel = rp.C <= (uint64_t)kHitBatch && opt.arms_kernel != 0 && (uint64_t)idx->n < (1ull << 42);
        for (int t = 1; t <= kTiers; ++t) {
            const TierShape &sh = shape(t);
            const bool usable = sh.kernel != TierKernel::none && !(arms_kernel && rp.C > (uint64_t)sh.hits);
            tier_cap[t] = usable ? (uint32_t)((uint64_t)sh.cap() * (uint64_t)(sh.widen ? opt.*sh.widen : 100) / 100u) : 0u;
        }
        tier_cap[kTiers] = 0xFFFFFFFFu;
        if (arms_kernel)
            tier_cap[3] = std::min(std::max(shape(3).cap(), tier_cap[6]), tier_cap[3]);
        else
            tier_cap[6] = (rp.G >= 0xFFF0u || rp.C >= 0xFFF0u) ? 0u : tier_cap[6] * 7 / 5;
        PlaceParams pp;
        pp.long3 = pp.long3_big = pp.dense3 = pp.dense6 = 0;
        pp.stats = opt.debug ? 1u : 0u;
        pp.barren = opt.barren ? 1u : 0u;
        pp.seg_info = nullptr;
        const bool cluster_barren = opt.barren >= 2 && rp.M > (uint64_t)k;
        split_on = opt.split >= (sizeof(SlotT) == 4 ? 1 : 2) && arms_kernel && (opt.split_len == 0 || opt.split_len >= 64);
        if (cluster_barren || split_on) {
            RC_TRY(w.seg_info.reserve((size_t)n_seg * sizeof(uint2)));
            pp.seg_info = w.seg_info.as<uint2>();
        }
        d_split = nullptr;
        if (split_on) {
            RC_TRY(w.split_buf.reserve(kSplitBytes));
            d_split = w.split_buf.as<char>();
            HIP_TRY(hipMemsetAsync(d_split, 0, 64, s));
        }
        pp.k = (uint32_t)k;
        pp.step = (uint32_t)step;
        pp.G = rp.G;
        pp.M = rp.M;
        for (int t = 1; t < kTiers; ++t) pp.cap[t - 1] = tier_cap[t];
        if (arms_kernel) {
            pp.long3 = (uint32_t)opt.long3;
            pp.long3_big = pp.long3 / 4u;
            pp.dense3 = (uint32_t)opt.dense3;
            pp.dense6 = (uint32_t)opt.dense6;
            if (force_tier == 3) {
                pp.long3 = pp.long3_big = 1;
                pp.dense3 = pp.dense6 = 0;
            }
            pp.cap[0] = (uint32_t)std::min<int64_t>(opt.cap1, shape(1).cap());
        }
        int force_eff = force_tier;
        while (force_eff > 1 && force_eff < kTiers && !tier_enabled(force_eff)) ++force_eff;
        pp.sum1 = kTier1MaxSum;
        pp.force_tier = force_eff;
        {
            uint32_t *long_list = w.ovf_list.as<uint32_t>();
            seg_stats_lanes_kernel<<<(unsigned)std::min<uint64_t>((n_seg + 63) / 64, 256ull * 9ull * 2ull), 64, 0, s>>>(
                rp, p_filt, seg_list, d_ctr + CT_SEG, kbuf, vbuf, pp, long_list, d_ctr);
            seg_stats_kernel<<<(unsigned)std::min<uint64_t>(n_seg, 256ull * 16ull), 64, 0, s>>>(
                rp, p_filt, seg_list, d_ctr + CT_LONGSEG, long_list, kbuf, vbuf, pp, d_ctr);
        }
        HIP_TRY(hipGetLastError());
        HIP_TRY(hipStreamWaitEvent(s, cx.ev[EV_HIT_ROWS], 0));
        if (cluster_barren) {
            HIP_TRY(hipEventRecord(cx.ev[EV_BARREN], s));
            cluster_barren_kernel<SlotT, 16384><<<256 * 32, 64, 0, s>>>(rp, pp, row_off, hits, seg_list, d_ctr + CT_SEG, kbuf, 1u, 1024u,
                                                                       d_ctr + CT_CLUSTER_CUR, d_ctr);
            HIP_TRY(hipEventRecord(cx.ev[EV_BARREN_SMALL], s));
            cluster_barren_kernel<SlotT, 131072><<<256 * 9, 64, 0, s>>>(rp, pp, row_off, hits, seg_list, d_ctr + CT_SEG, kbuf, 1025u,
                                                                       16384u, d_ctr + CT_CLUSTER_CUR + 1, d_ctr);
            HIP_TRY(hipGetLastError());
            HIP_TRY(hipEventRecord(cx.ev[EV_BARREN_BIG], s));
        }
        if (split_on) {
            SplitParams sp{};
            sp.range_len = (uint32_t)opt.split_len;
            sp.warm = (uint32_t)opt.split_warm;
            sp.min_span = (uint32_t)std::min<int64_t>(opt.split_min, 0x7FFFFFFF);
            sp.max_runs = kMaxRuns - kMaxSplits;
            sp.max_cuts = kMaxCuts;
            sp.max_splits = kMaxSplits;
            {
                BlockedSeg *const h_blocked = reinterpret_cast<BlockedSeg *>(h_split + kOffBlocked);
                std::lock_guard<std::mutex> lk(idx->mu);
                for (auto b = idx->split_blocked.rbegin(); b != idx->split_blocked.rend(); ++b)
                    for (int32_t p_ = 0; p_ < n_passes && sp.n_blocked < kSplitBlockedMax; ++p_)
                        if (b->sig == call_sig && ((rp.modes >> (8 * p_)) & 0xFFu) == (uint32_t)(b->key >> 32) &&
                            (uint32_t)b->key >= lo_lim && (uint32_t)b->key < hi_lim)
                            h_blocked[sp.n_blocked++] = BlockedSeg{(uint32_t)p_ * K + ((uint32_t)b->key - lo_lim), b->range_len, b->allowed, b->warm};
            }
            sp.blocked = reinterpret_cast<const BlockedSeg *>(d_split + kOffBlocked);
            if (sp.n_blocked)
                HIP_TRY(hipMemcpyAsync(d_split + kOffBlocked, h_split + kOffBlocked, (size_t)sp.n_blocked * sizeof(BlockedSeg), hipMemcpyHostToDevice, s));
            SplitChoice *const d_choice = reinterpret_cast<SplitChoice *>(d_split + kOffChoice);
            if (!sp.range_len) {
                HIP_TRY(hipMemsetAsync(d_choice, 0, sizeof(SplitChoice), s));
                split_tally_kernel<<<grid_for(n_seg), 256, 0, s>>>(rp, d_ctr + CT_SEG, kbuf, pp.seg_info, d_choice);
                split_pick_kernel<<<1, 1, 0, s>>>(d_choice, (uint32_t)opt.split_runs);
            }
            plan_ranges_kernel<<<grid_for(n_seg), 256, 0, s>>>(rp, sp, p_filt, seg_list, d_ctr + CT_SEG, kbuf, pp.seg_info,
                                                              reinterpret_cast<unsigned long long *>(d_split),
                                                              reinterpret_cast<RangeRun *>(d_split + kOffRuns),
                                                              reinterpret_cast<uint2 *>(d_split + kOffCuts),
                                                              reinterpret_cast<SplitSeg *>(d_split + kOffSplits), d_choice);
            HIP_TRY(hipGetLastError());
            HIP_TRY(hipMemcpyAsync(h_split, d_split, kOffMeta, hipMemcpyDeviceToHost, s));
        }
        if (opt.debug >= 2 && pp.seg_info) {
            unsigned long long *d_top = nullptr, h_top[2 * kTiers] = {};
            HIP_TRY(hipMalloc(&d_top, sizeof(h_top)));
            (void)hipMemsetAsync(d_top, 0, sizeof(h_top), s);
            top_uncut_kernel<<<grid_for(n_seg), 256, 0, s>>>(d_ctr + CT_SEG, kbuf, pp.seg_info, d_top);
            (void)hipMemcpyAsync(h_top, d_top, sizeof(h_top), hipMemcpyDeviceToHost, s);
            (void)hipStreamSynchronize(s);
            for (int t = 0; t < 2 * kTiers; ++t) {
                if (!h_top[t]) continue;
                uint2 info{};
                uint32_t g0 = 0;
                const size_t sj = (size_t)(h_top[t] & 0xFFFFFFFFull);
                (void)hipMemcpy(&info, pp.seg_info + sj, sizeof(info), hipMemcpyDeviceToHost);
                (void)hipMemcpy(&g0, seg_list + sj, sizeof(g0), hipMemcpyDeviceToHost);
                fprintf(stderr, "[asgart] tier %d, run whole, the segment with the most %s: at probe %u, %u probe positions%s, %u hits\n", t / 2 + 1,
                        t % 2 ? "hits" : "probe positions", g0, info.y & 0x7FFFFFFFu, (info.y >> 31) ? "" : " (cut short by the window)", info.x);
            }
            (void)hipFree(d_top);
        }
        order = nullptr;
        const uint32_t *sorted_keys = nullptr;
        RC_TRY(sort_segments(w, kbuf, vbuf, n_seg, s, &order, &sorted_keys, false));
        tier_bounds_kernel<<<1, 64, 0, s>>>(sorted_keys, d_ctr + CT_SEG, d_ctr);
        HIP_TRY(hipGetLastError());
        HIP_TRY(hipMemcpyAsync(h_ctr, d_ctr, kCtrBytes, hipMemcpyDeviceToHost, s));
        RC_TRY(wd_sync(idx, cx, s, "the hit rows and the placement of the segments"));
        seg_off[0] = 0;
        for (int t = 0; t < kTiers; ++t) {
            n_t[t] = h_ctr[CT_N1 + t];
            seg_off[t + 1] = seg_off[t] + n_t[t];
            h_tp[t] = h_ctr[CT_TPROBES1 + t];
            h_th[t] = h_ctr[CT_THITS1 + t];
        }
        h_split_hdr = reinterpret_cast<const unsigned long long *>(h_split);
        n_runs = split_on ? (uint32_t)h_split_hdr[0] : 0u;
        n_cuts = split_on ? (uint32_t)h_split_hdr[1] : 0u;
        n_splits = split_on ? (uint32_t)h_split_hdr[2] : 0u;
        split_segs.assign(n_splits, SplitSeg{});
        if (n_splits) memcpy(split_segs.data(), h_split + kOffSplits, (size_t)n_splits * sizeof(SplitSeg));
        n_split_segments = n_splits;
        if (opt.debug && split_on)
            for (const SplitSeg &sg : split_segs)
                fprintf(stderr, "[asgart] ranges: segment at probe %u: tier %u, %u probe positions, %u hits -> %u ranges\n", sg.g_seg0, sg.tier, sg.span,
                        sg.hits, sg.n_ranges);
        if (opt.debug && split_on)
            fprintf(stderr, "[asgart] %u long segment(s) cut into ranges: %u runs (ranges of %llu probes%s), %u cuts to check\n",
                    n_splits, n_runs, (unsigned long long)h_split_hdr[4], opt.split_len ? "" : ": the shortest that keeps the runs within the budget", n_cuts);
        if (opt.debug) {
            fprintf(stderr, "[asgart] %llu segments, %llu walked wave by wave; per tier:", (unsigned long long)n_seg,
                    (unsigned long long)h_ctr[CT_LONGSEG]);
            unsigned long long placed = 0;
            for (int t = 0; t < kTiers; ++t) {
                fprintf(stderr, " %llu", (unsigned long long)n_t[t]);
                placed += n_t[t];
            }
            fprintf(stderr, "; %llu barren (no arm can reach min_duplication_length: not run), %llu of them by the positions of their hits\n",
                    (unsigned long long)n_seg - placed, (unsigned long long)h_ctr[CT_CLUSTER_BARREN]);
            if (cluster_barren) {
                float ms_a = 0.f, ms_b = 0.f, ms_p = 0.f;
                (void)hipEventElapsedTime(&ms_a, cx.ev[EV_BARREN], cx.ev[EV_BARREN_SMALL]);
                (void)hipEventElapsedTime(&ms_b, cx.ev[EV_BARREN_SMALL], cx.ev[EV_BARREN_BIG]);
                (void)hipEventElapsedTime(&ms_p, cx.ev[EV_FILL], cx.ev[EV_BARREN]);
                fprintf(stderr, "[asgart] hit rows filled, placement walk beside it: %.2f ms; barren by position: segments of up to 1 024 hits %.2f ms, up to 16 384 hits %.2f ms\n",
                        ms_p, ms_a, ms_b);
            }
        }
        for (int t = 0; t < kTiers; ++t) ovf[t] = w.ovf_list.as<uint32_t>() + (size_t)t * (n_seg + 1);
        heavy_cap64 = (std::max<uint64_t>((uint64_t)rp.C * ((uint64_t)rp.tstar + 1u) + 64u, 4096u) + 3u) & ~3ull;
        if (heavy_cap64 >= (1ull << 24)) {
            set_error("max_cardinality * (max_gap_size / step + 1) = %llu live arms per segment: more than 2^24 are not supported",
                      (unsigned long long)heavy_cap64);
            return ASGART_E_CAP;
        }
        const size_t per_wg7 = (size_t)heavy_cap64 * (4 * sizeof(SlotT) + 28);
        const size_t per_wg6 = (size_t)caph * (4 * sizeof(SlotT) + 16);
        const size_t per_wg = std::max(per_wg6, per_wg7);
        n_wg7 = (unsigned)std::max<uint64_t>(1, std::min<uint64_t>(256, (16ull << 30) / (4 * per_wg)));
        region = std::max(per_wg6 * 256, per_wg * (size_t)n_wg7);
        RC_TRY(w.scratch.reserve(region * 4));
        scratch6 = w.scratch.as<char>();
        scratch7 = scratch6 + region;
        return 0;
    }

    struct WorkList {
        const uint32_t *list;
        const unsigned long long *count;
        unsigned long long *cursor;
        int ovf_into;
        uint32_t cap_limit;
        char *scratch = nullptr;
    };
    uint32_t test_cap() const { return opt.test_cap_limit >= 0 ? (uint32_t)opt.test_cap_limit : 0xFFFFFFFFu; }

    template <int T, int SET>
    static void launch_shape(const ExtParams<SlotT> &p, unsigned grid, hipStream_t st) {
        constexpr TierShape sh = Tiers::shape[T][SET];
        constexpr int cap = (int)sh.cap();
        if constexpr (sh.kernel == TierKernel::wave)
            extend_kernel<SlotT, cap><<<grid, sh.threads, 0, st>>>(p);
        else if constexpr (sh.kernel == TierKernel::fast)
            extend_fast_kernel<SlotT, sh.layers, sh.threads, sh.hits, sh.rows, 2><<<grid, sh.threads, 0, st>>>(p);
        else if constexpr (sh.kernel == TierKernel::k8)
            extend_k8_kernel<SlotT, sh.layers, sh.threads, sh.hits, sh.rows, 2, T == 0><<<grid, sh.threads, 0, st>>>(p);
        else if constexpr (sh.kernel != TierKernel::none)
            extend_heavy_kernel<SlotT, cap, sh.threads, (int)sh.kernel - (int)TierKernel::heavy_lds><<<grid, sh.threads, 0, st>>>(p);
    }
    template <int... I>
    static void launch_entry(int entry, std::integer_sequence<int, I...>, const ExtParams<SlotT> &p, unsigned grid, hipStream_t st) {
        ((entry == I ? launch_shape<I / 2, I % 2>(p, grid, st) : void()), ...);
    }

    int32_t launch_kernel(int tier, const WorkList &wl, uint64_t n_items, hipStream_t st) {
        const bool runs = tier == 0;
        if (shape(tier).kernel == TierKernel::none) {
            set_error("internal: tier %d has no kernel in this set, its %llu work items would be lost", tier, (unsigned long long)n_items);
            return ASGART_E_CAP;
        }
        const uint32_t stat = runs ? (uint32_t)kRunsStat : (uint32_t)tier;
        ExtParams<SlotT> p = base;
        p.runs = runs ? reinterpret_cast<const RangeRun *>(d_split + kOffRuns) : nullptr;
        p.run_meta = runs ? reinterpret_cast<uint32_t *>(d_split + kOffMeta) : nullptr;
        p.run_dump = runs ? w.split_dump.as<uint32_t>() : nullptr;
        p.seg_list = wl.list;
        p.n_seg_ptr = wl.count;
        p.cursor = wl.cursor;
        p.ovf_list = runs || wl.ovf_into >= kTiers ? nullptr : ovf[wl.ovf_into - 1];
        p.ovf_count = d_ctr + CT_OVF1 + wl.ovf_into - 1;
        p.scratch = wl.scratch && tier >= 6 ? wl.scratch : tier == kTiers ? scratch7 : scratch6;
        p.cap_limit = wl.cap_limit;
        p.tier = stat;
        p.seg_slots = w.seg_slots.as<unsigned long long>() + (size_t)4096 * (size_t)(stat & 7);
        p.hb = cx.d_hb ? cx.d_hb + (size_t)2 * SearchCtx::kHbSlots * (size_t)(stat & 7) : nullptr;
        uint64_t g = runs ? n_items : tier == kTiers ? (uint64_t)n_wg7 : (uint64_t)shape(tier).grid;
        if (!runs && opt.grid[tier] > 0) g = tier >= 3 ? std::min<uint64_t>(g, (uint64_t)opt.grid[tier]) : (uint64_t)opt.grid[tier];
        launch_entry(2 * tier + (arms_kernel ? 0 : 1), std::make_integer_sequence<int, 2 * (kTiers + 1)>{}, p,
                     (unsigned)std::min<uint64_t>(n_items, g), st);
        return 0;
    }

// ... 283 lines not shown
                HIP_TRY(hipMemsetAsync(d_ctr + CT_CURF, 0, 8, s));
                RC_TRY(launch_kernel(Tiers::kRunsTier, WorkList{reinterpret_cast<const uint32_t *>(d_split + kOffAgain), d_ctr + CT_NF,
                                                                d_ctr + CT_CURF, Tiers::kRunsTier, test_cap()}, n_again, s));
                HIP_TRY(hipGetLastError());
            }
            HIP_TRY(hipMemcpyAsync(h_ctr, d_ctr, kCtrBytes, hipMemcpyDeviceToHost, s));
            RC_TRY(wd_sync(idx, cx, s, "the ranges of the cut segments"));
        }
        return 0;
    }

    unsigned long long tier_sum(int ct1, int t) const { return h_ctr[ct1 + t - 1] + (t == Tiers::kRunsTier ? h_ctr[ct1 + kRunsStat - 1] : 0ull); }
    unsigned long long tier_longest(int t) const { return std::max(h_ctr[CT_SEGMAX1 + t - 1], t == Tiers::kRunsTier ? h_ctr[CT_SEGMAX1 + kRunsStat - 1] : 0ull); }
    static const TierShape &stat_shape(int t) { return Tiers::shape[t][0]; }

    int32_t finish_tiers() {
        PROF_DUMP("concurrent tiers");
        if (opt.debug) {
            fprintf(stderr, "[asgart] all tiers and early re-runs done %.1f ms after the launches\n", since_launch());
            double tot = 0.0;
            fprintf(stderr, "[asgart] compute-unit time held per tier (CU-ms; workgroups):");
            for (int t = 1; t <= kTiers; ++t) {
                const double cu_ms = (double)tier_sum(CT_BUSY1, t) * 1e-5 / stat_shape(t).wg_per_cu;
                tot += cu_ms;
                fprintf(stderr, " %d: %.0f (%llu)", t, cu_ms, tier_sum(CT_WGS1, t));
            }
            fprintf(stderr, "  total %.0f = %.1f ms of the whole chip\n", tot, tot / 256.0);
            fprintf(stderr, "[asgart] per tier: hit-probes / hits per hit-probe / CU-microseconds per hit-probe:");
            for (int t = 1; t <= kTiers; ++t) {
                const double hp = (double)h_tp[t - 1];
                fprintf(stderr, " %d: %.0fK / %.1f / %.2f", t, hp / 1e3, hp > 0 ? (double)h_th[t - 1] / hp : 0.0,
                        hp > 0 ? (double)tier_sum(CT_BUSY1, t) * 1e-2 / stat_shape(t).wg_per_cu / hp : 0.0);
            }
            fprintf(stderr, "\n");
        }
        {
            float longest = 0.f;
            for (int t = 1; t <= kTiers; ++t) {
                float ms = 0.f;
                if (!tier_ran[t]) continue;
                if (hipEventElapsedTime(&ms, cx.ev[EV_TIERS], cx.tier_ev[t - 1]) == hipSuccess) longest = std::max(longest, ms);
                else (void)hipGetLastError();
            }
            ms_longest_tier = longest;
        }
        n_overflow = 0;
        for (int t = 1; t < kTiers; ++t) n_overflow += h_ctr[CT_OVF1 + t - 1];
        if (opt.debug) {
            fprintf(stderr, "[asgart] overflow out of tiers 1..%d:", kTiers - 1);
            for (int t = 1; t < kTiers; ++t) fprintf(stderr, " %llu", (unsigned long long)h_ctr[CT_OVF1 + t - 1]);
            fprintf(stderr, "\n");
        }
        n_heavy = 0;
        for (int t = 3; t <= kTiers; ++t) n_heavy += n_t[t - 1];
        const auto t_casc0 = std::chrono::steady_clock::now();
        for (int src = 1; src < kTiers; ++src) {
            const uint64_t skip = early_n[src];
            const uint64_t n_ovf = h_ctr[CT_OVF1 + src - 1] - skip;
            if (!n_ovf) continue;
            const int dst = next_holding_more(src);
            *h_scalar = n_ovf;
            HIP_TRY(hipMemcpyAsync(d_ctr + CT_NF, h_scalar, 8, hipMemcpyHostToDevice, s));
            HIP_TRY(hipMemsetAsync(d_ctr + CT_CURF, 0, 8, s));
            RC_TRY(launch_kernel(dst, WorkList{ovf[src - 1] + skip, d_ctr + CT_NF, d_ctr + CT_CURF, dst, 0xFFFFFFFFu}, n_ovf, s));
            HIP_TRY(hipGetLastError());
            HIP_TRY(hipMemcpyAsync(h_ctr, d_ctr, kCtrBytes, hipMemcpyDeviceToHost, s));
            RC_TRY(wd_sync(idx, cx, s, "a re-run of overflowed segments"));
            PROF_DUMP("cascade");
        }
        ms_tier2 = std::chrono::duration<double, std::milli>(std::chrono::steady_clock::now() -
                                                             t_casc0).count();
        if (h_ctr[CT_OVF1 + kTiers - 1]) {
            set_error("internal: %llu segment(s) overflowed the last extension tier (%llu arm slots)",
                      (unsigned long long)h_ctr[CT_OVF1 + kTiers - 1], (unsigned long long)heavy_cap64);
            return ASGART_E_CAP;
        }
        ms_longest_segment = 0.0;
        for (int t = 0; t < kRunsStat; ++t) ms_longest_segment = std::max(ms_longest_segment, (double)h_ctr[CT_SEGMAX1 + t] * 1e-5);
        if (opt.debug) {
            fprintf(stderr, "[asgart] longest single segment per tier (ms):");
            for (int t = 1; t <= kTiers; ++t) fprintf(stderr, " %d: %.2f", t, (double)tier_longest(t) * 1e-5);
            fprintf(stderr, "\n");
        }
        remember_plan_estimates();
        return 0;
    }

    void plan_estimates(double *est) const {
        const bool known = cx.plan_known && cx.plan_sig == call_sig;
        for (int t = 0; t <= kTiers; ++t) est[t] = known && cx.plan_est[t] > 0.0 ? cx.plan_est[t] : stat_shape(t).profile_ms;
    }
    void remember_plan_estimates() {
        if (!(cx.plan_known && cx.plan_sig == call_sig))
            for (double &e : cx.plan_est) e = 0.0;
        cx.plan_sig = call_sig;
        cx.plan_known = true;
        for (int t = 1; t <= kTiers; ++t) {
            if (!tier_ran[t]) continue;
            const double seg = (double)h_ctr[CT_SEGMAX1 + t - 1] * 1e-5;
            const TierShape &sh = stat_shape(t);
            const double spread = (double)h_ctr[CT_BUSY1 + t - 1] * 1e-5 / sh.wg_per_cu / std::min(256.0, (double)sh.grid / sh.wg_per_cu);
            cx.plan_est[t] = std::max(seg, spread);
        }
        float runs = 0.f;
        if (n_runs) {
            if (hipEventElapsedTime(&runs, cx.ev[EV_TIERS], cx.runs_ev) != hipSuccess) {
                (void)hipGetLastError();
                runs = 0.f;
            }
            cx.plan_est[0] = runs;
        }
    }

    int32_t records() {
        HIP_TRY(hipEventRecord(cx.ev[EV_EXTENDED], s));
        const uint64_t n_rec = h_ctr[CT_SD];
        if (n_rec) {
            void *hp = nullptr;
            RC_TRY(cx.pinned((size_t)n_rec * sizeof(SdRec), &hp));
            h_recs = static_cast<const SdRec *>(hp);
            n_hrec = (size_t)n_rec;
        }
        if (n_rec) {
            RC_TRY(sort_records(w, w.fam_sds.as<SdRec>(), n_rec, s));
            HIP_TRY(hipMemcpyAsync(const_cast<SdRec *>(h_recs), w.rec_sorted.p, (size_t)n_rec * sizeof(SdRec),
                                   hipMemcpyDeviceToHost, s));
        }
        const auto t_post0 = std::chrono::steady_clock::now();
        RC_TRY(wd_sync(idx, cx, s, "the ordering of the records"));
        const auto t_post1 = std::chrono::steady_clock::now();
        using Part = SearchCtx::FamPart;
        auto assemble = [&](size_t b0, size_t b1, Part &out) {
            int32_t pass = 0;
            for (size_t f0 = b0; f0 < b1;) {
                if (h_recs[f0].g_start == kVoidStart) break;
                size_t f1 = f0;
                while (f1 < n_hrec && h_recs[f1].g_start == h_recs[f0].g_start && h_recs[f1].fam_seq == h_recs[f0].fam_seq) ++f1;
                while (pass + 1 < n_passes && h_recs[f0].g_start >= (uint32_t)(pass + 1) * K) ++pass;
                if (h_recs[f1 - 1].create_seq != kTombstone) {
                    std::vector<asgart_proto_sd> &sds = out.sds[pass];
                    for (size_t j = f0; j < f1; ++j) {
                        if (j > f0 && h_recs[j].create_seq == h_recs[j - 1].create_seq) continue;
                        sds.push_back(h_recs[j].sd);
                    }
                    out.ends[pass].push_back(sds.size());
                    out.keys[pass].push_back(((uint64_t)(lo_lim + (h_recs[f0].g_start - (uint32_t)pass * K)) << 32) |
                                             (uint64_t)h_recs[f0].fam_seq);
                }
                f0 = f1;
            }
        };
        const size_t n_parts = n_hrec >= (1u << 17) ? 4 : 1;
        size_t bound[5] = {0, 0, 0, 0, n_hrec};
        for (size_t t = 1; t < n_parts; ++t) {
            size_t b = std::max(bound[t - 1], n_hrec * t / n_parts);
            while (b > 0 && b < n_hrec && h_recs[b].g_start == h_recs[b - 1].g_start && h_recs[b].fam_seq == h_recs[b - 1].fam_seq) ++b;
            bound[t] = b;
        }
        for (size_t t = n_parts; t < 4; ++t) bound[t] = n_hrec;
        std::vector<Part> &parts = cx.fam_parts;
        parts.resize(4);
        for (size_t t = 0; t < 4; ++t)
            for (int32_t p = 0; p < 4; ++p) {
                parts[t].sds[p].clear();
                parts[t].ends[p].clear();
                parts[t].keys[p].clear();
                if (t < n_parts && p < n_passes)
                    parts[t].sds[p].reserve((bound[t + 1] - bound[t]) / (size_t)n_passes + (bound[t + 1] - bound[t]) / 4 + 16);
            }
        {
            std::vector<std::thread> workers;
            for (size_t t = 1; t < n_parts; ++t) workers.emplace_back([&, t]() { assemble(bound[t], bound[t + 1], parts[t]); });
            assemble(bound[0], bound[1], parts[0]);
            for (auto &th : workers) th.join();
        }
        for (int32_t p = 0; p < n_passes; ++p) {
            asgart_families *const fo = fams[p];
            size_t tot = 0, nf = 0;
            for (const Part &pt : parts) {
                tot += pt.sds[p].size();
                nf += pt.ends[p].size();
            }
            if (!tot && !nf) continue;
            fo->sds.reserve(fo->sds.size() + tot);
            fo->fam_offsets.reserve(fo->fam_offsets.size() + nf);
            fo->fam_keys.reserve(fo->fam_keys.size() + nf);
            for (const Part &pt : parts) {
                const size_t at = fo->sds.size();
                fo->sds.insert(fo->sds.end(), pt.sds[p].begin(), pt.sds[p].end());
                for (uint64_t e : pt.ends[p]) fo->fam_offsets.push_back(at + e);
                fo->fam_keys.insert(fo->fam_keys.end(), pt.keys[p].begin(), pt.keys[p].end());
            }
        }
        if (opt.debug)
// ... 456 lines not shown
    std::vector<std::vector<uint64_t>> prog((size_t)n_passes, std::vector<uint64_t>((size_t)std::max<int64_t>(n_chunks, 1), 0));
    std::vector<std::atomic<int>> finished((size_t)n_passes);
    for (auto &f : finished) f.store(0);
    auto searched = [&](int32_t p) {
        if (finished[p].load(std::memory_order_acquire)) return true;
        const volatile uint64_t *pr = prog[p].data();
        for (int64_t c = 0; c < n_chunks; ++c)
            if (pr[c]) return true;
        return false;
    };
    std::lock_guard<std::mutex> pass_lock(idx->pass_mu);
    struct Owns {
        Owns() { asgart::tl_owns_pass_mu = true; }
        ~Owns() { asgart::tl_owns_pass_mu = false; }
    } owns;
    while ((int32_t)idx->pass_workers.size() + 1 < n_passes) idx->pass_workers.emplace_back(new asgart::PassWorker());
    auto body = [&](int32_t p) {
            if (p > 0)
                while (!searched(p - 1)) std::this_thread::sleep_for(std::chrono::microseconds(100));
            const int32_t j = order[p];
            asgart_families *f = new (std::nothrow) asgart_families();
            if (!f) {
                rcs[p] = ASGART_E_OOM;
                errs[p] = "out of host memory";
            } else {
                rcs[p] = run_search(idx, chunks, n_chunks, &settings[j], shard, n_shards, false, f, nullptr, nullptr,
                                    nullptr, prog[p].data());
                if (rcs[p] != 0) {
                    errs[p] = asgart_last_error();
                    delete f;
                } else {
                    fams[p] = f;
                }
            }
            finished[p].store(1, std::memory_order_release);
    };
    for (int32_t p = 1; p < n_passes; ++p) idx->pass_workers[(size_t)p - 1]->submit([&body, p]() { body(p); });
    body(0);
    for (int32_t p = 1; p < n_passes; ++p) idx->pass_workers[(size_t)p - 1]->wait();
    for (int32_t p = 0; p < n_passes; ++p)
        if (rcs[p] != 0) {
            for (auto *f : fams) delete f;
            set_error("pass %d of %d: %s", order[p], n_passes, errs[p].c_str());
            return rcs[p];
        }
    for (int32_t p = 0; p < n_passes; ++p) out[order[p]] = fams[p];
    timed.ok = true;
    return 0;
}

void asgart_families_counts(const asgart_families *f, uint64_t *n_families, uint64_t *n_sds) {
    if (n_families) *n_families = f ? f->fam_offsets.size() - 1 : 0;
    if (n_sds) *n_sds = f ? f->sds.size() : 0;
}

void asgart_families_copy(const asgart_families *f, uint64_t *fam_offsets, asgart_proto_sd *sds) {
    if (!f) return;
    if (fam_offsets) memcpy(fam_offsets, f->fam_offsets.data(), f->fam_offsets.size() * 8);
    if (sds && !f->sds.empty()) memcpy(sds, f->sds.data(), f->sds.size() * sizeof(asgart_proto_sd));
}

void asgart_families_keys(const asgart_families *f, uint64_t *keys) {
    if (f && keys && !f->fam_keys.empty()) memcpy(keys, f->fam_keys.data(), f->fam_keys.size() * 8);
}

void asgart_families_free(asgart_families *f) { delete f; }

int64_t asgart_probe_hits(asgart_index *idx, const uint64_t *chunks, int64_t n_chunks,
                          const asgart_settings *settings, uint8_t *status, uint64_t *row_offsets,
                          uint64_t *hits, uint64_t *n_hits) {
    std::vector<uint8_t> st;
    std::vector<uint64_t> ro, hv;
    int32_t rc = run_search(idx, chunks, n_chunks, settings, 0, 1, true, nullptr, &st, &ro, &hv, nullptr);
    if (rc != 0) return rc;
    if (n_hits) *n_hits = hv.size();
    if (status) {
        if (!st.empty()) memcpy(status, st.data(), st.size());
        memcpy(row_offsets, ro.data(), ro.size() * 8);
        if (!hv.empty()) memcpy(hits, hv.data(), hv.size() * 8);
    }
    return (int64_t)st.size();
}

int32_t asgart_get_stats(asgart_index *idx, uint32_t flags, asgart_stats *out) {
    if (!idx || !out) {
        set_error("bad argument");
        return ASGART_E_ARG;
    }
    idx->acquire_all();
    const int sel = (int)((flags >> 8) & 0xFFu);
    SearchCtx &cx = idx->ctx[sel >= 1 && sel <= kNumCtx ? sel - 1 : idx->last_ctx];
    int32_t rc = [&]() -> int32_t {
        if ((flags & (ASGART_STATS_YARDSTICK | ASGART_STATS_RAW_HITS)) && cx.has_last && cx.last_P && !cx.raw_done) {
            REFUSE_POISONED(idx);
            HIP_TRY(hipSetDevice(idx->device));
            unsigned long long *d_ctr = cx.ws.counters.as<unsigned long long>();
            hipStream_t s = cx.stream;
            const RunParams &rp = cx.last_rp;
            HIP_TRY(hipMemsetAsync(d_ctr + CT_RAW_HITS, 0, 8, s));
            const unsigned g_raw = std::min<uint32_t>(rp.n_tiles(1024u), 256u * 16u);
            if (idx->wide)
                raw_hits_kernel<uint64_t><<<g_raw, 256, 0, s>>>(idx->view<uint64_t>(), rp, cx.ws.p_filt.as<uint32_t>() - rp.g_lo,
                                                                cx.ws.p_raw.as<uint32_t>() - rp.g_lo, d_ctr + CT_RAW_HITS);
            else
                raw_hits_kernel<uint32_t><<<g_raw, 256, 0, s>>>(idx->view<uint32_t>(), rp, cx.ws.p_filt.as<uint32_t>() - rp.g_lo,
                                                                cx.ws.p_raw.as<uint32_t>() - rp.g_lo, d_ctr + CT_RAW_HITS);
            HIP_TRY(hipGetLastError());
            unsigned long long v = 0;
            HIP_TRY(read_back(&v, d_ctr + CT_RAW_HITS, 8, s));
            cx.stats.raw_hits = v;
            cx.raw_done = true;
        }
        if ((flags & ASGART_STATS_YARDSTICK) && cx.has_last && cx.last_P) {
            REFUSE_POISONED(idx);
            HIP_TRY(hipSetDevice(idx->device));
            unsigned long long *d_ctr = cx.ws.counters.as<unsigned long long>();
            hipStream_t s = cx.stream;
            HIP_TRY(hipMemsetAsync(d_ctr + CT_BISECT, 0, 8, s));
            RunParams rp = cx.last_rp;
            for (uint32_t p = 0; p < rp.n_passes && p < 4u; ++p) {
                rp.pbits[p] = idx->opt.posbits ? idx->d_pbits[rp.mode_of_pass(p)] : nullptr;
                if ((rp.blank >> p) & 1u) rp.pbits[p] = nullptr;
            }
            const unsigned g = rp.n_tiles(256u);
            if (idx->wide)
                yardstick_kernel<uint64_t><<<g, 256, 0, s>>>(idx->view<uint64_t>(), rp,
                                                             cx.ws.p_filt.as<uint32_t>() - rp.g_lo, d_ctr);
            else
                yardstick_kernel<uint32_t><<<g, 256, 0, s>>>(idx->view<uint32_t>(), rp,
                                                             cx.ws.p_filt.as<uint32_t>() - rp.g_lo, d_ctr);
            HIP_TRY(hipGetLastError());
            HIP_TRY(hipMemsetAsync(d_ctr + CT_ALG_BYTES, 0, 16, s));
            HIP_TRY(hipMemsetAsync(d_ctr + CT_ALG_BYTES16, 0, 8, s));
            const unsigned gp = rp.n_tiles((uint32_t)kProbeBlock);
            auto account = [&](auto slot_tag) {
                using SlotT = decltype(slot_tag);
                IndexView<SlotT> ix = idx->view<SlotT>();
                probe_count_kernel<SlotT, true><<<gp, kProbeThreads, 0, s>>>(
                    ix, rp, nullptr, nullptr, nullptr, nullptr, nullptr, d_ctr);
                big_count_kernel<SlotT, true><<<2048, 256, 0, s>>>(
                    ix, rp, cx.ws.p_lo.as<SlotT>() - rp.g_lo, cx.ws.p_raw.as<uint32_t>() - rp.g_lo, nullptr,
                    cx.ws.big_list.as<uint32_t>(), d_ctr);
                if (ix.sap)
                    rank_count_kernel<SlotT, true><<<2048, 256, 0, s>>>(
                        ix, rp, cx.ws.p_lo.as<SlotT>() - rp.g_lo, cx.ws.p_raw.as<uint32_t>() - rp.g_lo, nullptr,
                        cx.ws.rank_list.as<uint32_t>(), nullptr, d_ctr);
            };
            if (idx->wide) account(uint64_t{}); else account(uint32_t{});
            HIP_TRY(hipGetLastError());
            unsigned long long v = 0, ab[2] = {0, 0}, a16 = 0;
            HIP_TRY(read_back(&v, d_ctr + CT_BISECT, 8, s));
            HIP_TRY(read_back(ab, d_ctr + CT_ALG_BYTES, 16, s));
            HIP_TRY(read_back(&a16, d_ctr + CT_ALG_BYTES16, 8, s));
            cx.stats.bisect_steps = v;
            cx.stats.search_bytes = ab[0];
            cx.stats.probes_filter_rejected = ab[1];
            cx.stats.search_bytes_wide_loads = a16;
        }
        *out = cx.stats;
        return 0;
    }();
    idx->release_all();
    return rc;
}

}
// ... 1 lines not shown
```

asgart_amd/csrc/pipeline_dev.hpp:

```cpp
#pragma once

#include "extend_common_dev.hpp"

namespace asgart {

constexpr int kProbeBlock = 256;
constexpr int kProbeThreads = 64;
constexpr int kProbeSub = kProbeBlock / kProbeThreads;
constexpr int kMaxHalf = (kMaxKey + 1) / 2;
constexpr int kWinBytes = ((kProbeBlock + 2) * kMaxHalf + 15 + 16 + 15) / 16 * 16;

template <class SlotT, bool COUNT>
__global__ __launch_bounds__(kProbeThreads) void probe_count_kernel(IndexView<SlotT> ix, RunParams rp,
                                                                    SlotT *__restrict__ p_lo,
                                                                    uint32_t *__restrict__ p_raw,
                                                                    uint32_t *__restrict__ p_filt,
                                                                    uint32_t *__restrict__ big_list,
                                                                    uint32_t *__restrict__ rank_list,
                                                                    unsigned long long *__restrict__ ctr) {
    __shared__ __attribute__((aligned(16))) uint8_t s_text[kWinBytes];
    __shared__ uint32_t s_half[kProbeBlock + 2];
    constexpr int kPbLoads = (kProbeBlock * kMaxHalf + 127) / 128 + 2;
    __shared__ __attribute__((aligned(16))) uint32_t s_pb[kPbLoads * 4];
    __shared__ uint8_t s_surv[kProbeBlock];
// ... 772 lines not shown
    const uint64_t lo = p_lo[g];
    unsigned long long w = row_off[g];
    for (uint32_t r = 0; r < raw; ++r) {
        const SlotT x = ix.sa[lo + r];
        if (keep_hit(x, i, s, L, (rp.mode_of(c) & 2u) != 0u)) hits[w++] = x;
    }
}

template <class SlotT>
__global__ __launch_bounds__(256) void fill_big_kernel(IndexView<SlotT> ix, RunParams rp,
                                                       const SlotT *__restrict__ p_lo,
                                                       const uint32_t *__restrict__ p_raw,
                                                       const uint32_t *__restrict__ p_filt,
                                                       const unsigned long long *__restrict__ row_off,
                                                       SlotT *__restrict__ hits,
                                                       const uint32_t *__restrict__ big_list,
                                                       const unsigned long long *__restrict__ ctr) {
    const uint32_t lane = threadIdx.x & 63u;
    const unsigned long long lt_mask = (1ull << lane) - 1ull;
    const uint64_t n_big = ctr[CT_BIG];
    const uint64_t wave = ((uint64_t)blockIdx.x * blockDim.x + threadIdx.x) >> 6;
    const uint64_t n_waves = ((uint64_t)gridDim.x * blockDim.x) >> 6;
    for (uint64_t e0 = wave * 64u; e0 < n_big; e0 += n_waves * 64u) {
        const uint32_t np = (uint32_t)min((uint64_t)64, n_big - e0);
        unsigned long long s = 0, L = 0, i = 0, lo = 0, hi = 0, w0 = 0;
        uint32_t md = 0;
        bool want = false;
        if (lane < np) {
            const uint32_t g = big_list[e0 + lane];
            const uint32_t f = p_filt[g];
            want = f != 0 && f < kPending;
            if (want) {
                const int c = chunk_of(rp.ch, g);
                md = rp.mode_of(c);
                s = rp.ch.start[c];
                L = rp.ch.len[c];
                i = (unsigned long long)(g - rp.ch.pbase[c] + 1) * (unsigned long long)rp.step;
                lo = p_lo[g];
                hi = lo + p_raw[g];
                w0 = row_off[g];
            }
        }
        unsigned long long todo = __ballot(want);
        while (todo) {
            const uint32_t p = (uint32_t)(__ffsll((long long)todo) - 1);
            todo &= todo - 1;
            const unsigned long long lo_p = lane_of(lo, p), hi_p = lane_of(hi, p), i_p = lane_of(i, p),
                                     s_p = lane_of(s, p), L_p = lane_of(L, p);
            const bool rev_p = (lane_of(md, p) & 2u) != 0u;
            unsigned long long w = lane_of(w0, p);
            for (unsigned long long base = lo_p; base < hi_p; base += 256) {
                SlotT x[4];
#pragma unroll
                for (int u = 0; u < 4; ++u) {
                    const unsigned long long r = base + 64u * u + lane;
                    x[u] = r < hi_p ? ix.sa[r] : (SlotT)0;
                }
#pragma unroll
                for (int u = 0; u < 4; ++u) {
                    const unsigned long long r = base + 64u * u + lane;
                    const bool keep = r < hi_p && keep_hit(x[u], i_p, s_p, L_p, rev_p);
                    const unsigned long long m = __ballot(keep);
                    if (keep) hits[w + __popcll(m & lt_mask)] = x[u];
                    w += __popcll(m);
                }
            }
        }
    }
}

struct PlaceParams {
    uint32_t cap[kTiers - 1];
    uint32_t sum1;
    int force_tier;
    uint32_t long3;
    uint32_t long3_big;
    uint32_t dense6;
    uint32_t stats;
    uint32_t barren;
    uint2 *seg_info;
    uint32_t k, step, G;
    unsigned long long M;
    uint32_t dense3;
};

constexpr int kTierBarren = kTiers + 1;
__device__ inline bool segment_is_barren(const PlaceParams &pp, uint32_t n_hit, uint32_t span_probes) {
    if (!pp.barren || n_hit == 0u) return false;
    const unsigned long long len_left_max = (unsigned long long)span_probes * pp.step + pp.k;
    const unsigned long long thr_max = max((unsigned long long)pp.G, len_left_max / 10ull);
    return (unsigned long long)pp.k + (unsigned long long)(n_hit - 1u) * (thr_max + pp.k - 1ull) < pp.M;
}

__device__ inline uint32_t placement_key(int tier, unsigned long long sum, uint32_t g0) {
    uint32_t low;
    if (tier == 1) {
        low = sum >= 1024ull ? 1023u - (uint32_t)min(sum >> 5, 1023ull) : 1024u + (g0 >> 4);
    } else {
        const uint32_t s29 = sum > 0x1FFFFFFFull ? 0x1FFFFFFFu : (uint32_t)sum;
        low = 0x1FFFFFFFu - s29;
    }
    return (((uint32_t)tier - 1u) << 29) | low;
}

__device__ inline int place_tier(uint32_t bound, unsigned long long sum, uint32_t n_probes, const PlaceParams &pp) {
    if (bound <= pp.cap[0] && sum <= pp.sum1) return 1;
    if (pp.long3 && bound <= pp.cap[2] &&
        (n_probes >= pp.long3 || (bound > pp.cap[4] && n_probes >= pp.long3_big))) {
        if (!pp.dense3 || sum >= (unsigned long long)pp.dense3 * n_probes || bound > pp.cap[5]) return 3;
        return 6;
    }
    for (int t = 2; t < kTiers; ++t) {
        if (t == 3 && pp.long3) continue;
        if (bound <= pp.cap[t - 1]) {
            if (t == 6 && pp.dense6 && bound <= pp.cap[2] && sum >= (unsigned long long)pp.dense6 * n_probes) return 3;
            return t;
        }
    }
    return kTiers;
}

constexpr uint32_t kLaneWalk = 256;

__global__ __launch_bounds__(64) void seg_stats_lanes_kernel(RunParams rp, const uint32_t *__restrict__ p_filt,
                                                             const uint32_t *__restrict__ seg_list,
                                                             const unsigned long long *__restrict__ n_seg_ptr,
                                                             uint32_t *__restrict__ keys,
                                                             uint32_t *__restrict__ vals, PlaceParams pp,
                                                             uint32_t *__restrict__ long_list,
                                                             unsigned long long *__restrict__ ctr) {
    __shared__ uint32_t s_ring[65 * 64];
    const uint32_t lane = threadIdx.x;
    const uint64_t n_seg = *n_seg_ptr;
    const uint32_t RW = min(rp.tstar, 64u) + 1u;
    for (uint64_t base = (uint64_t)blockIdx.x * 64u; base < n_seg; base += (uint64_t)gridDim.x * 64u) {
        const uint64_t sidx = base + lane;
        const bool have = sidx < n_seg;
        uint32_t g0 = 0, g_end = 0;
        bool window_cut = false;
        if (have) {
            g0 = seg_list[sidx];
            const uint32_t chunk_end = rp.ch.pbase[chunk_of(rp.ch, g0) + 1];
            g_end = min(chunk_end, rp.win_end(g0));
            window_cut = g_end < chunk_end;
        }
        for (uint32_t r = 0; r < RW; ++r) s_ring[r * 64u + lane] = 0;
        uint32_t quiet = 0, mx = 0, bound = 0, n_probes = 0, wsum = 0, head = 0, steps = 0, g = g0, n_hit = 0;
        unsigned long long sum = 0;
        bool done = !have, by_quiet = false;
        while (!done && g < g_end && steps < kLaneWalk) {
            const uint32_t f = p_filt[g];
            ++g;
            ++steps;
            const bool hit = f >= 1u && f < kPending;
            if (!hit && f != 0u) continue;
            if (!hit) {
                if (++quiet >= rp.tstar) {
                    done = true;
                    by_quiet = true;
                    break;
                }
            } else {
                quiet = 0;
            }
            const uint32_t v = hit ? f : 0u;
            ++n_probes;
            n_hit += hit ? 1u : 0u;
            const uint32_t at = head * 64u + lane;
            wsum += v - s_ring[at];
            s_ring[at] = v;
            head = head + 1u == RW ? 0u : head + 1u;
            bound = max(bound, wsum);
            mx = max(mx, v);
            sum += v;
        }
        if (g >= g_end) done = true;
        if (have && done) {
            if (rp.tstar > 64u) bound = 0xFFFFFFFFu;
            int tier = place_tier(bound, sum, n_probes, pp);
            if (mx > 1 && pp.force_tier > tier) tier = min(pp.force_tier, kTiers);
            if ((by_quiet || !window_cut) && segment_is_barren(pp, n_hit, g - g0)) tier = kTierBarren;
            keys[sidx] = placement_key(tier, sum, g0);
            vals[sidx] = g0;
            if (pp.seg_info)
                pp.seg_info[sidx] = make_uint2(sum > 0xFFFFFFFFull ? 0xFFFFFFFFu : (uint32_t)sum,
                                               (g - g0) | ((by_quiet || !window_cut) ? 0x80000000u : 0u));
            if (pp.stats) {
                atomicAdd(&ctr[CT_TPROBES1 + tier - 1], (unsigned long long)n_hit);
                atomicAdd(&ctr[CT_THITS1 + tier - 1], sum);
            }
        }
        const unsigned long long lm = __ballot(have && !done);
        if (lm) {
            const int leader = __ffsll((long long)lm) - 1;
            unsigned long long at = 0;
            if ((int)lane == leader) at = atomicAdd(&ctr[CT_LONGSEG], (unsigned long long)__popcll(lm));
            at = __shfl(at, leader);
            if (have && !done) long_list[at + __popcll(lm & ((1ull << lane) - 1ull))] = (uint32_t)sidx;
        }
    }
}

__global__ __launch_bounds__(64) void seg_stats_kernel(RunParams rp, const uint32_t *__restrict__ p_filt,
                                                       const uint32_t *__restrict__ seg_list,
                                                       const unsigned long long *__restrict__ n_ptr,
                                                       const uint32_t *__restrict__ idx_list,
                                                       uint32_t *__restrict__ keys,
                                                       uint32_t *__restrict__ vals, PlaceParams pp,
                                                       unsigned long long *__restrict__ ctr) {
    __shared__ uint32_t s_ext[64 + 64];
    const int lane = threadIdx.x;
    const unsigned long long lt_mask = (1ull << lane) - 1ull;
    const uint64_t n_items = *n_ptr;
    const uint32_t TW = min(rp.tstar, 64u);
    for (uint64_t item = blockIdx.x; item < n_items; item += gridDim.x) {
        const uint64_t sidx = idx_list ? (uint64_t)idx_list[item] : item;
        const uint32_t g0 = seg_list[sidx];
        const int c = chunk_of_uniform(rp.ch, g0);
        const uint32_t g_end = min(rp.ch.pbase[c + 1], rp.win_end(g0));
        const bool window_cut = g_end < rp.ch.pbase[c + 1];
        uint32_t quiet = 0, mx = 0, bound = 0, n_probes = 0, n_hit = 0, g_stop = g_end, g_after_hit = g0 + 1u;
        unsigned long long sum = 0;
        bool done = false;
        s_ext[lane] = 0;
        lds_barrier();
        uint32_t f_next = g0 + (uint32_t)lane < g_end ? p_filt[g0 + lane] : kSkipN;
        for (uint32_t g = g0; g < g_end && !done; g += 64) {
            const uint32_t f = f_next;
            f_next = g + 64u + (uint32_t)lane < g_end ? p_filt[g + 64u + lane] : kSkipN;
            const unsigned long long hm = __ballot(f >= 1u && f < kPending);
            const unsigned long long qm = __ballot(f == 0u);
            if (!(hm | qm)) continue;
            unsigned long long live = ~0ull;
            {
                const unsigned long long hb = hm & lt_mask;
                const int lh = hb ? 63 - __clzll((long long)hb) : -1;
                const unsigned long long above_lh = lh < 0 ? ~0ull : (lh == 63 ? 0ull : ~((2ull << lh) - 1ull));
                const uint32_t run = (uint32_t)__popcll(qm & (lt_mask | (1ull << lane)) & above_lh) + (lh < 0 ? quiet : 0u);
                const unsigned long long term = __ballot(((qm >> lane) & 1ull) && run >= rp.tstar);
                if (term) {
                    const uint32_t pos = (uint32_t)(__shfl(lh, __ffsll((long long)term) - 1) + 1);
                    done = true;
                    g_stop = pos ? g + pos : g_after_hit;
                    live = (1ull << pos) - 1ull;
                } else {
                    const int last = hm ? 63 - __clzll((long long)hm) : -1;
                    if (last >= 0) g_after_hit = g + (uint32_t)last + 1u;
                    const unsigned long long above = last < 0 ? ~0ull : (last == 63 ? 0ull : ~((2ull << last) - 1ull));
                    quiet = (uint32_t)__popcll(qm & above) + (last < 0 ? quiet : 0u);
                }
            }
            const unsigned long long procm = (hm | qm) & live;
            const bool proc = (procm >> lane) & 1ull;
            const uint32_t v = ((hm & live) >> lane) & 1ull ? f : 0u;
            const uint32_t r = (uint32_t)__popcll(procm & lt_mask);
            const uint32_t n_proc = (uint32_t)__popcll(procm);
            n_probes += n_proc;
            n_hit += (uint32_t)__popcll(hm & live);
            if (proc) s_ext[TW + r] = v;
            lds_barrier();
            uint32_t wsum = 0;
            if (proc)
                for (uint32_t d = 0; d <= TW; ++d) wsum += s_ext[TW + r - d];
            uint32_t m = v, wm = wsum;
            unsigned long long sv = v;
            for (int off = 32; off > 0; off >>= 1) {
                sv += __shfl_down(sv, off);
                m = max(m, (uint32_t)__shfl_down(m, off));
                wm = max(wm, (uint32_t)__shfl_down(wm, off));
            }
            sum += __shfl(sv, 0);
            mx = max(mx, (uint32_t)__shfl(m, 0));
            bound = max(bound, (uint32_t)__shfl(wm, 0));
            const uint32_t keep = (uint32_t)lane < TW ? s_ext[n_proc + lane] : 0u;
            lds_barrier();
            if ((uint32_t)lane < TW) s_ext[lane] = keep;
            lds_barrier();
        }
        if (rp.tstar > 64u) bound = 0xFFFFFFFFu;
        if (lane == 0) {
            int tier = place_tier(bound, sum, n_probes, pp);
            if (mx > 1 && pp.force_tier > tier) tier = min(pp.force_tier, kTiers);
            if ((done || !window_cut) && segment_is_barren(pp, n_hit, min(g_stop, g_end) - g0)) tier = kTierBarren;
            keys[sidx] = placement_key(tier, sum, g0);
            vals[sidx] = g0;
            if (pp.seg_info)
                pp.seg_info[sidx] = make_uint2(sum > 0xFFFFFFFFull ? 0xFFFFFFFFu : (uint32_t)sum,
                                               (min(g_stop, g_end) - g0) | ((done || !window_cut) ? 0x80000000u : 0u));
            if (pp.stats) {
                atomicAdd(&ctr[CT_TPROBES1 + tier - 1], (unsigned long long)n_hit);
                atomicAdd(&ctr[CT_THITS1 + tier - 1], sum);
            }
        }
        lds_barrier();
    }
}

template <class PosT, int BITS>
__global__ __launch_bounds__(64) void cluster_barren_kernel(RunParams rp, PlaceParams pp,
                                                            const unsigned long long *__restrict__ row_off,
                                                            const PosT *__restrict__ hits,
                                                            const uint32_t *__restrict__ seg_list,
                                                            const unsigned long long *__restrict__ n_seg_ptr,
                                                            uint32_t *__restrict__ keys, uint32_t min_hits, uint32_t max_hits,
                                                            unsigned long long *__restrict__ cursor,
                                                            unsigned long long *__restrict__ ctr) {
    static_assert((BITS & (BITS - 1)) == 0 && BITS >= 2048, "bitmap size");
    constexpr uint32_t kWords = BITS / 32, kShift = 32 - __builtin_ctz((unsigned)BITS);
    __shared__ uint32_t s_bits[kWords];
    const uint32_t lane = threadIdx.x;
    const uint64_t n_seg = *n_seg_ptr;
    uint32_t n_barren = 0;
    auto bit_of = [&](uint32_t b) { return (b * 2654435761u) >> kShift; };
    for (;;) {
        unsigned long long base = 0;
        if (lane == 0) base = atomicAdd(cursor, 64ull);
        base = lane_of(base, 0u);
        if (base >= n_seg) break;
        const uint64_t sj = base + lane;
        bool cand = false;
        uint32_t key_l = 0, span_l = 0;
        unsigned long long lo_l = 0, hi_l = 0;
        if (sj < n_seg) {
            key_l = keys[sj];
            const uint2 info = pp.seg_info[sj];
            span_l = info.y & 0x7FFFFFFFu;
            cand = (key_l >> 29) < (uint32_t)kTiers && (info.y >> 31) && info.x >= min_hits && info.x <= max_hits;
            if (cand) {
                const uint32_t g0 = seg_list[sj];
                lo_l = row_off[g0];
                hi_l = row_off[g0 + span_l];
                cand = hi_l > lo_l && hi_l - lo_l <= (unsigned long long)max_hits;
            }
        }
        unsigned long long todo = __ballot(cand);
        while (todo) {
            const uint32_t l = (uint32_t)(__ffsll((long long)todo) - 1);
            todo &= todo - 1ull;
            const uint32_t key = lane_of(key_l, l), span = lane_of(span_l, l);
            const unsigned long long lo = lane_of(lo_l, l);
            const uint32_t n = (uint32_t)(lane_of(hi_l, l) - lo);
            const unsigned long long len_left_max = (unsigned long long)span * pp.step + pp.k;
            const unsigned long long thr_max = max((unsigned long long)pp.G, len_left_max / 10ull);
            const unsigned long long w = thr_max + pp.k;
            const unsigned long long need = (pp.M - pp.k) / w + 1ull;
            if (need < 2ull || need > 64ull) continue;
            const double inv_w = 1.0 / (double)w;
            auto bucket_of = [&](unsigned long long x) -> uint32_t {
                unsigned long long q = (unsigned long long)((double)x * inv_w);
                const long long r = (long long)(x - q * w);
                q += r >= (long long)w ? 1ull : 0ull;
                q -= r < 0 ? 1ull : 0ull;
                return (uint32_t)q;
            };
            for (uint32_t j = lane; j < kWords; j += 64u) s_bits[j] = 0u;
            __builtin_amdgcn_wave_barrier();
            __asm__ volatile("s_waitcnt lgkmcnt(0)" ::: "memory");
            for (uint32_t j0 = 0; j0 < n; j0 += 512u) {
                PosT xv[8];
#pragma unroll
                for (int u = 0; u < 8; ++u) {
                    const uint32_t j = j0 + (uint32_t)u * 64u + lane;
                    xv[u] = j < n ? hits[lo + j] : (PosT)0;
                }
#pragma unroll
                for (int u = 0; u < 8; ++u) {
// ... 314 lines not shown
```

include/asgart_hip.h:

```cpp
#ifndef ASGART_HIP_H
#define ASGART_HIP_H

#include <stdint.h>

#ifdef __cplusplus
extern "C" {
#endif

#define ASGART_OK 0
#define ASGART_E_ARG (-1)
#define ASGART_E_OOM (-2)
#define ASGART_E_HIP (-3)
#define ASGART_E_CAP (-4)

typedef struct asgart_settings {
    uint64_t probe_size;
    uint32_t max_gap_size;
    uint64_t min_duplication_length;
    uint64_t max_cardinality;
    uint8_t reverse;
    uint8_t complement;
} asgart_settings;

typedef struct asgart_proto_sd {
    uint64_t left, right, left_length, right_length;
} asgart_proto_sd;

typedef struct asgart_stats {
    double ms_total;
    double ms_search;
    double ms_scan;
    double ms_fill;
    double ms_extend;
    uint64_t probes_total;
    uint64_t probes_n_skipped;
    uint64_t probes_searched;
    uint64_t probes_card_skipped;
    uint64_t probes_with_hits;
    uint64_t raw_hits;
    uint64_t filtered_hits;
    uint64_t segments;
    uint64_t families;
    uint64_t proto_sds;
    uint64_t bisect_steps;
    uint64_t search_launches;
    uint64_t overflow_segments;
    double ms_extend_tier2;
    uint64_t heavy_segments;
    double ms_probe_count;
    uint64_t search_bytes;
    uint64_t probes_filter_rejected;
    uint64_t search_bytes_wide_loads;
    double ms_longest_tier;
    uint64_t passes;
    double ms_longest_segment;
    uint64_t split_segments;
    uint64_t split_refused;
} asgart_stats;

typedef struct asgart_index asgart_index;
typedef struct asgart_families asgart_families;

int32_t asgart_sa_build64(const uint8_t *T, int64_t *SA, int64_t n);

int32_t asgart_index_create(const uint8_t *T, int64_t n, const int64_t *SA, int64_t sa_len,
                            int32_t device, asgart_index **out);
void asgart_index_destroy(asgart_index *idx);

int32_t asgart_index_clone(asgart_index *src, int32_t device, asgart_index **out);

int32_t asgart_index_export(asgart_index *idx, const void **d_text, const void **d_sa, int32_t *sa_entry_bytes);
int32_t asgart_index_create_device(const void *d_text, int64_t n, const void *d_sa, int64_t sa_len,
                                   int32_t sa_entry_bytes, int32_t device, asgart_index **out);

int32_t asgart_prepare_data(const uint8_t *const *records, const uint64_t *record_lens, int64_t n_records,
                            int32_t skip_masked, int32_t device, uint8_t *text_out, uint64_t *chunks,
                            int64_t chunks_cap, int64_t *n_chunks, asgart_index **index_out);

int64_t asgart_trim_cache(int32_t device);

int32_t asgart_debug_dump_stacks(void);

int32_t asgart_index_create_trim(const uint8_t *T, int64_t n, const int64_t *SA, int64_t sa_len,
                                 int64_t trim_start, int64_t trim_end, int32_t device,
                                 asgart_index **out);

int32_t asgart_index_set_option(asgart_index *idx, const char *name, int64_t value);

int64_t asgart_index_check_sa(asgart_index *idx);

int32_t asgart_index_prepare(asgart_index *idx, uint64_t probe_size);

int32_t asgart_search_duplications(asgart_index *idx, const uint64_t *chunks, int64_t n_chunks,
                                   const asgart_settings *settings, volatile uint64_t *progress,
                                   asgart_families **out);

int32_t asgart_search_duplications_shard(asgart_index *idx, const uint64_t *chunks,
                                         int64_t n_chunks, const asgart_settings *settings,
                                         int32_t shard, int32_t n_shards,
                                         asgart_families **out);

int32_t asgart_search_duplications_multi(asgart_index *const *indices, int32_t n_devices,
                                         const uint64_t *chunks, int64_t n_chunks,
                                         const asgart_settings *settings, volatile uint64_t *progress,
                                         asgart_families **out);

int32_t asgart_search_duplications_ex(asgart_index *idx, const uint64_t *chunks, int64_t n_chunks,
                                      const asgart_settings *settings, int32_t shard, int32_t n_shards,
                                      volatile uint64_t *progress, asgart_families **out);

int32_t asgart_search_duplications_passes(asgart_index *idx, const uint64_t *chunks, int64_t n_chunks,
                                          const asgart_settings *settings, int32_t n_passes,
                                          asgart_families **out);
int32_t asgart_search_duplications_passes_shard(asgart_index *idx, const uint64_t *chunks, int64_t n_chunks,
                                                const asgart_settings *settings, int32_t n_passes,
                                                int32_t shard, int32_t n_shards, asgart_families **out);

void asgart_families_counts(const asgart_families *f, uint64_t *n_families, uint64_t *n_sds);
void asgart_families_copy(const asgart_families *f, uint64_t *fam_offsets, asgart_proto_sd *sds);
void asgart_families_keys(const asgart_families *f, uint64_t *keys);
void asgart_families_free(asgart_families *f);

int32_t asgart_compute_scores(asgart_index *idx, const asgart_proto_sd *sds, int64_t n_sd,
                              int32_t reversed, int32_t complemented, float *identity);

int32_t asgart_score_owners(const asgart_proto_sd *sds, int64_t n_sd, int32_t n_shards, int32_t *owner);
int32_t asgart_score_costs(const asgart_proto_sd *sds, int64_t n_sd, uint64_t *cost);

int32_t asgart_tier_plan(int32_t budget, const uint64_t *n_work, int64_t tier_order, const double *est_ms, double main_ms,
                         int32_t *stream_of, int32_t *launch);

int64_t asgart_compute_scores_shard(asgart_index *idx, const asgart_proto_sd *sds, int64_t n_sd,
                                    int32_t reversed, int32_t complemented, int32_t shard, int32_t n_shards,
                                    float *identity);

int32_t asgart_compute_scores_multi(asgart_index *const *indices, int32_t n_devices, const asgart_proto_sd *sds,
                                    int64_t n_sd, int32_t reversed, int32_t complemented, float *identity);

int32_t asgart_compute_scores_flags(asgart_index *idx, const asgart_proto_sd *sds, const uint8_t *flags, int64_t n_sd,
                                    float *identity);
int64_t asgart_compute_scores_flags_shard(asgart_index *idx, const asgart_proto_sd *sds, const uint8_t *flags,
                                          int64_t n_sd, int32_t shard, int32_t n_shards, float *identity);
int32_t asgart_compute_scores_flags_multi(asgart_index *const *indices, int32_t n_devices, const asgart_proto_sd *sds,
                                          const uint8_t *flags, int64_t n_sd, float *identity);

int32_t asgart_post_process(asgart_index *idx, const uint64_t *fam_offsets, uint64_t n_families,
                            const asgart_proto_sd *sds, int32_t threads, asgart_families **out);

typedef struct asgart_source asgart_source;
int32_t asgart_source_create(const uint8_t *const *records, const uint64_t *record_lens, int64_t n_records,
                             int32_t device, asgart_source **out);
void asgart_source_destroy(asgart_source *src);
int32_t asgart_extract_sequences(asgart_source *src, const asgart_proto_sd *sds, const uint8_t *flags, int64_t n_sd,
                                 int64_t first, uint8_t *out, uint64_t out_cap, uint64_t *seq_ends, int64_t *n_done);

typedef struct asgart_fasta asgart_fasta;
typedef struct asgart_fasta_record {
    uint64_t file;
    uint64_t header_offset;
    uint64_t header_len;
    uint64_t start;
    uint64_t len;
} asgart_fasta_record;
int32_t asgart_fasta_read(const uint8_t *const *files, const uint64_t *file_lens, int64_t n_files, int32_t skip_masked,
                          int32_t device, asgart_fasta **out);
int32_t asgart_fasta_counts(const asgart_fasta *f, int64_t *n_records, int64_t *n_chunks, uint64_t *n_text);
int32_t asgart_fasta_copy(const asgart_fasta *f, asgart_fasta_record *records, uint64_t *chunks, uint8_t *text);
int32_t asgart_fasta_read_text(const asgart_fasta *f, uint64_t lo, uint64_t hi, uint8_t *out);
int32_t asgart_fasta_index(asgart_fasta *f, asgart_index **out);
int32_t asgart_fasta_source(asgart_fasta *f, asgart_source **out);
void asgart_fasta_free(asgart_fasta *f);
int32_t asgart_fasta_timings(const asgart_fasta *f, double *ms4);
void asgart_fasta_geometry(uint64_t *tile_bytes, uint64_t *piece_bytes, uint64_t *vector_bytes);


int32_t asgart_searcher_cache_get(asgart_index *idx, const uint8_t *patterns8, int64_t n_pat,
                                  uint64_t *lo, uint64_t *hi);
int32_t asgart_searcher_search(asgart_index *idx, const uint8_t *patterns, int64_t n_pat,
                               uint64_t k, uint64_t *lo, uint64_t *hi);
int32_t asgart_sa_read(asgart_index *idx, uint64_t lo, uint64_t hi, int64_t *out);

int64_t asgart_probe_hits(asgart_index *idx, const uint64_t *chunks, int64_t n_chunks,
                          const asgart_settings *settings, uint8_t *status,
                          uint64_t *row_offsets, uint64_t *hits, uint64_t *n_hits);

#define ASGART_STATS_YARDSTICK 1u
#define ASGART_STATS_RAW_HITS 2u
#define ASGART_STATS_CTX(i) (((uint32_t)(i) + 1u) << 8)
int32_t asgart_get_stats(asgart_index *idx, uint32_t flags, asgart_stats *out);

const char *asgart_last_error(void);
const char *asgart_version(void);

#ifdef __cplusplus
}
#endif
#endif
```

Before: 43880.

## Promote hit-heavy segments from small tiers to the next larger tier

Adds a tail-up rule to tier placement: segments in fast tiers 2, 4 or 5 whose hit sum exceeds a threshold move to the next enabled tier with a larger capacity. This targets long-tail segments that stall small workgroups. The rule is on by default when fewer tier streams exist than resident tiers, and the default threshold is set only for 32-bit slots. It also retunes the per-tier profile estimates, folds the thresholds into the plan signature, and raises single-workgroup tier estimates to a chip-wide busy bound for scheduling. The risk is overloading the larger tiers.

```diff
diff --git a/asgart_amd/__init__.py b/asgart_amd/__init__.py
--- a/asgart_amd/__init__.py
+++ b/asgart_amd/__init__.py
@@ -31,6 +31,7 @@
     "asgart_compute_scores_flags", "asgart_compute_scores_flags_shard", "asgart_compute_scores_flags_multi",
     "asgart_fasta_read", "asgart_fasta_counts", "asgart_fasta_copy", "asgart_fasta_read_text", "asgart_fasta_index",
     "asgart_fasta_source", "asgart_fasta_free", "asgart_fasta_timings", "asgart_fasta_geometry",
+    "asgart_index_set_tail_up", "asgart_tier_segments", "asgart_tier_profile",
 )
 
 
@@ -205,6 +206,13 @@
     L.asgart_probe_hits.restype = C.c_int64
     L.asgart_get_stats.argtypes = [vp, C.c_uint32, C.POINTER(Stats)]
     L.asgart_get_stats.restype = C.c_int32
+    if hasattr(L, "asgart_tier_segments"):
+        L.asgart_index_set_tail_up.argtypes = [vp, C.c_int32, C.c_int64]
+        L.asgart_index_set_tail_up.restype = C.c_int32
+        L.asgart_tier_segments.argtypes = [vp, vp]
+        L.asgart_tier_segments.restype = C.c_int32
+        L.asgart_tier_profile.argtypes = [vp, vp]
+        L.asgart_tier_profile.restype = C.c_int32
     L.asgart_last_error.argtypes = []
     L.asgart_last_error.restype = C.c_char_p
     L.asgart_version.argtypes = []
@@ -347,6 +355,14 @@
 
     def set_option(self, name: str, value: int):
         _check(load_library().asgart_index_set_option(self._h, name.encode(), int(value)))
+
+    def set_tail_up(self, mode: int, hits: int = 0):
+        _check(load_library().asgart_index_set_tail_up(self._h, int(mode), int(hits)))
+
+    def tier_segments(self) -> Tuple[np.ndarray, int]:
+        out = np.zeros(8, dtype=np.uint64)
+        _check(load_library().asgart_tier_segments(self._h, _ptr(out)))
+        return out[:7].copy(), int(out[7])
 
     def check_sa(self) -> int:
         r = int(load_library().asgart_index_check_sa(self._h))
@@ -607,6 +623,13 @@
     return stream_of, launch
 
 
+def tier_profile() -> Tuple[np.ndarray, np.ndarray]:
+    ms = np.zeros(8, dtype=np.float64)
+    hits = np.zeros(8, dtype=np.uint64)
+    _check(load_library().asgart_tier_profile(_ptr(ms), _ptr(hits)))
+    return ms, hits
+
+
 def compute_scores_multi(indices: Sequence[Index], sds: np.ndarray, reversed_: bool = False,
                          complemented: bool = False) -> np.ndarray:
     L = load_library()
diff --git a/asgart_amd/csrc/device_base.hpp b/asgart_amd/csrc/device_base.hpp
--- a/asgart_amd/csrc/device_base.hpp
+++ b/asgart_amd/csrc/device_base.hpp
@@ -48,6 +48,7 @@
     CT_SEGMAX1 = 160,
     CT_CLUSTER_BARREN = 168,
     CT_CLUSTER_CUR = 169,
+    CT_TAIL_UP = 171,
     CT_COUNT = 176
 };
 
diff --git a/asgart_amd/csrc/extend_common_dev.hpp b/asgart_amd/csrc/extend_common_dev.hpp
--- a/asgart_amd/csrc/extend_common_dev.hpp
+++ b/asgart_amd/csrc/extend_common_dev.hpp
@@ -131,12 +131,23 @@
         atomicAdd(&P.ctr[CT_BUSY1 + P.tier - 1u], 0ull - wall_clock64());
     }
 }
+#ifdef ASGART_SEG_TOP
+constexpr unsigned long long kSegTopMin = 200000;
+constexpr uint32_t kSegTopWords = 512;
+#endif
 template <class PosT>
 __device__ inline void seg_clock(const ExtParams<PosT> &P, bool last = false) {
     if (!P.seg_slots || P.tier < 2u || P.tier > (uint32_t)kRunsStat) return;
     const unsigned long long now = wall_clock64();
     const unsigned long long prev = atomicExch(&P.seg_slots[blockIdx.x & 4095u], last ? 0ull : now);
     if (prev && now > prev) atomicMax(&P.ctr[CT_SEGMAX1 + P.tier - 1u], now - prev);
+#ifdef ASGART_SEG_TOP
+    if (prev && now > prev && now - prev >= kSegTopMin) {
+        unsigned long long *log = P.seg_slots - (size_t)4096 * (P.tier & 7u) + 4096 + (size_t)kSegTopWords * (P.tier & 7u);
+        const unsigned long long at = atomicAdd(log, 1ull);
+        if (at + 1u < kSegTopWords) log[1u + at] = now - prev;
+    }
+#endif
 }
 template <class PosT>
 __device__ inline void wg_busy(const ExtParams<PosT> &P) {
diff --git a/asgart_amd/csrc/index.hip b/asgart_amd/csrc/index.hip
--- a/asgart_amd/csrc/index.hip
+++ b/asgart_amd/csrc/index.hip
@@ -1157,6 +1157,7 @@
     idx->trim_end = src->trim_end;
     idx->wide = src->wide;
     idx->opt = src->opt;
+    idx->tail_up = src->tail_up;
     idx->h_tail = src->h_tail;
     for (auto &cx : idx->ctx) memset(&cx.stats, 0, sizeof(cx.stats));
     src->acquire_all();
@@ -1280,6 +1281,22 @@
     if (rc == 0 && !strcmp(name, "test_fail_alloc")) asgart::fail_alloc_countdown().store(value);
     idx->release_all();
     return rc;
+}
+
+int32_t asgart_index_set_tail_up(asgart_index *idx, int32_t mode, int64_t hits) {
+    if (!idx) {
+        set_error("index is NULL");
+        return ASGART_E_ARG;
+    }
+    if (mode < 0 || mode > 2 || hits < 0 || hits > (1ll << 31)) {
+        set_error("asgart_index_set_tail_up: mode %d outside [0, 2] or %lld hits outside [0, 2^31]", (int)mode, (long long)hits);
+        return ASGART_E_ARG;
+    }
+    idx->acquire_all();
+    idx->tail_up.mode = mode;
+    idx->tail_up.hits = hits;
+    idx->release_all();
+    return 0;
 }
 
 int64_t asgart_index_check_sa(asgart_index *idx) {
diff --git a/asgart_amd/csrc/index.hpp b/asgart_amd/csrc/index.hpp
--- a/asgart_amd/csrc/index.hpp
+++ b/asgart_amd/csrc/index.hpp
@@ -156,6 +156,7 @@
     double plan_est[8] = {};
     Workspace ws;
     asgart_stats stats;
+    uint64_t tier_segments[8] = {};
     RunParams last_rp;
     bool has_last = false;
     bool raw_done = false;
@@ -266,6 +267,10 @@
     int64_t test_stall_s = 0;
     int64_t watchdog_s = 120;
 };
+struct TailUp {
+    int32_t mode = 1;
+    int64_t hits = 0;
+};
 int32_t create_ctx_streams(SearchCtx &cx);
 int hw_queue_budget();
 int32_t tier_plan(int budget, const uint64_t *n_work, int64_t tier_order, const double *est_ms, double main_ms,
@@ -354,6 +359,7 @@
     std::atomic<bool> poisoned{false};
     double tail_ms[4] = {-1.0, -1.0, -1.0, -1.0};
     asgart::Options opt;
+    asgart::TailUp tail_up;
     asgart::SearchCtx ctx[asgart::kNumCtx];
     int last_ctx = 0;
     std::mutex mu;
diff --git a/asgart_amd/csrc/pipeline.hip b/asgart_amd/csrc/pipeline.hip
--- a/asgart_amd/csrc/pipeline.hip
+++ b/asgart_amd/csrc/pipeline.hip
@@ -7,6 +7,7 @@
 #include <algorithm>
 #include <atomic>
 #include <chrono>
+#include <functional>
 #include <string>
 #include <thread>
 #include <utility>
@@ -78,6 +79,8 @@
     int64_t Options::*widen;
     bool early;
     double profile_ms;
+    uint32_t tail_hits = 0;
+    double tail_profile_ms = 0.0;
     constexpr uint32_t cap() const { return (uint32_t)(layers * slots); }
 };
 template <class SlotT>
@@ -85,20 +88,20 @@
     static constexpr bool k32 = sizeof(SlotT) == 4;
     static constexpr int kLong = k32 ? 2048 : 1024;
     static constexpr TierShape kNone = {TierKernel::none, 0, 0, 0, 0, 0, 1, 0, nullptr, false, 0.0};
-    static constexpr TierShape kWave = {TierKernel::wave, 64, 1, 256, kHitBatch, 0, 11, 256 * 8, nullptr, false, 4.6};
-    static constexpr TierShape kHbm = {TierKernel::heavy_hbm, kHeavyThreads, 1, 1, kHitBatch, 0, 1, 256, nullptr, false, 33.0};
-    static constexpr TierShape kK8 = {TierKernel::k8, 1024, k32 ? 5 : 4, 896, kHitBatch, kLong, 1, 256, &Options::cap3_pct, true, 67.0};
+    static constexpr TierShape kWave = {TierKernel::wave, 64, 1, 256, kHitBatch, 0, 11, 256 * 8, nullptr, false, 3.4};
+    static constexpr TierShape kHbm = {TierKernel::heavy_hbm, kHeavyThreads, 1, 1, kHitBatch, 0, 1, 256, nullptr, false, 56.6};
+    static constexpr TierShape kK8 = {TierKernel::k8, 1024, k32 ? 5 : 4, 896, kHitBatch, kLong, 1, 256, &Options::cap3_pct, true, 56.6};
     static constexpr TierShape shape[kTiers + 1][2] = {
         {{kK8.kernel, kK8.threads, kK8.layers, kK8.slots, kK8.hits, kK8.rows, 1, 0, nullptr, false, 67.0}, kNone},
         {kWave, kWave},
         {{TierKernel::fast, 64, k32 ? 8 : 5, 64, 512, 256, 8, 256 * 8, nullptr, false, 51.8},
          {TierKernel::heavy_lds, kMidThreads, 1, 768, kHitBatch, 0, 3, 256 * 3, nullptr, false, 51.8}},
         {kK8, kNone},
-        {{TierKernel::fast, 256, k32 ? 4 : 2, 256, 512, 512, 4, 256 * 4, &Options::cap45_pct, false, 35.5},
+        {{TierKernel::fast, 256, k32 ? 4 : 2, 256, 512, 512, 4, 256 * 4, &Options::cap45_pct, false, 35.5, k32 ? 36000u : 0u, 8.7},
          {TierKernel::heavy_lds, kHeavyThreads, 1, k32 ? 2432 : 1664, kHitBatch, 0, 1, 256, nullptr, false, 35.5}},
         {{TierKernel::fast, 512, k32 ? 4 : 2, 512, kHitBatch, 1024, 2, 256 * 2, &Options::cap45_pct, false, 53.0}, kNone},
-        {{TierKernel::fast, 1024, k32 ? 5 : 4, 1024, kHitBatch, kLong, 1, 256, k32 ? &Options::cap6_pct : &Options::cap6w_pct, true, 33.0},
-         {TierKernel::heavy_hybrid, kHeavyThreads, 1, k32 ? 4608 : 3072, kHitBatch, 0, 1, 256, nullptr, true, 33.0}},
+        {{TierKernel::fast, 1024, k32 ? 5 : 4, 1024, kHitBatch, kLong, 1, 256, k32 ? &Options::cap6_pct : &Options::cap6w_pct, true, 56.6},
+         {TierKernel::heavy_hybrid, kHeavyThreads, 1, k32 ? 4608 : 3072, kHitBatch, 0, 1, 256, nullptr, true, 56.6}},
         {kHbm, kHbm},
     };
     static constexpr int kRunsTier = 3;
@@ -278,6 +281,7 @@
     const int64_t n_chunks;
     const uint64_t k, step, n;
     const Options opt;
+    const TailUp tail_up;
     static constexpr size_t kCtrBytes = (size_t)CT_COUNT * 8;
     static constexpr size_t kSplitMirror = 512 << 10;
     using Tiers = TierTable<SlotT>;
@@ -308,6 +312,7 @@
     size_t n_hrec = 0;
     bool arms_kernel = false, split_on = false;
     uint32_t tier_cap[kTiers + 1] = {};
+    uint32_t tail_hits[kTiers + 1] = {};
     char *d_split = nullptr;
     const uint32_t *order = nullptr;
     uint64_t n_t[kTiers] = {}, seg_off[kTiers + 1] = {};
@@ -334,17 +339,13 @@
           n_shards(n_shards_), want_csr(want_csr_), fams(fams_), status_out(status_out_), rowoff_out(rowoff_out_),
           hits_out(hits_out_), w(cx_.ws), s(cx_.stream), st(&sts_[0]), fam_out(fams_ != nullptr),
           n_chunks(n_chunks_pass_ * (int64_t)n_passes_), k(sts_[0].probe_size), step(sts_[0].probe_size / 2),
-          n((uint64_t)idx_->n), opt(idx_->opt) {}
+          n((uint64_t)idx_->n), opt(idx_->opt), tail_up(idx_->tail_up) {}
 
     uint32_t pass_of_probe(uint32_t g) const { return std::min<uint32_t>(g / K, (uint32_t)n_passes - 1u); }
     uint32_t pass_offset(uint32_t g) const { return lo_lim + (g - pass_of_probe(g) * K); }
     const TierShape &shape(int t) const { return Tiers::shape[t][arms_kernel ? 0 : 1]; }
     bool tier_enabled(int t) const { return t >= 1 && t <= kTiers && tier_cap[t] != 0; }
-    int next_holding_more(int src) const {
-        int dst = src + 1;
-        while (dst < kTiers && (!tier_enabled(dst) || tier_cap[dst] <= tier_cap[src])) ++dst;
-        return dst;
-    }
+    int next_holding_more(int src) const { return asgart::next_holding_more(tier_cap + 1, src); }
     double since_launch() const {
         return std::chrono::duration<double, std::milli>(std::chrono::steady_clock::now() - t_launch).count();
     }
@@ -619,6 +620,17 @@
             }
             pp.cap[0] = (uint32_t)std::min<int64_t>(opt.cap1, shape(1).cap());
         }
+        {
+            int n_resident = 0;
+            for (int t = 2; t < kTiers; ++t)
+                n_resident += tier_enabled(t) && (shape(t).kernel == TierKernel::fast || shape(t).kernel == TierKernel::k8) ? 1 : 0;
+            const bool on = tail_up.mode == 2 || (tail_up.mode == 1 && cx.n_tier_st < n_resident);
+            for (int t = 1; t < kTiers; ++t) {
+                const bool source = (t == 2 || t == 4 || t == 5) && shape(t).kernel == TierKernel::fast;
+                const uint32_t thr = !source ? 0u : tail_up.hits > 0 ? (uint32_t)std::min<int64_t>(tail_up.hits, 0xFFFFFFFFll) : shape(t).tail_hits;
+                pp.tail_hits[t - 1] = tail_hits[t] = on && tier_enabled(t) ? thr : 0u;
+            }
+        }
         int force_eff = force_tier;
         while (force_eff > 1 && force_eff < kTiers && !tier_enabled(force_eff)) ++force_eff;
         pp.sum1 = kTier1MaxSum;
@@ -694,6 +706,20 @@
                         t % 2 ? "hits" : "probe positions", g0, info.y & 0x7FFFFFFFu, (info.y >> 31) ? "" : " (cut short by the window)", info.x);
             }
             (void)hipFree(d_top);
+            std::vector<uint32_t> h_keys((size_t)n_seg);
+            std::vector<uint2> h_info((size_t)n_seg);
+            (void)hipMemcpy(h_keys.data(), kbuf, (size_t)n_seg * 4, hipMemcpyDeviceToHost);
+            (void)hipMemcpy(h_info.data(), pp.seg_info, (size_t)n_seg * sizeof(uint2), hipMemcpyDeviceToHost);
+            for (uint32_t t = 1; t < (uint32_t)kTiers; ++t) {
+                std::vector<uint32_t> rich;
+                for (size_t sj = 0; sj < (size_t)n_seg; ++sj)
+                    if (h_keys[sj] >> 29 == t) rich.push_back(h_info[sj].x);
+                const size_t top = std::min<size_t>(rich.size(), 48);
+                std::partial_sort(rich.begin(), rich.begin() + top, rich.end(), std::greater<uint32_t>());
+                fprintf(stderr, "[asgart] tier %u, run whole, the most hits:", t + 1);
+                for (size_t i = 0; i < top; ++i) fprintf(stderr, " %u", rich[i]);
+                fprintf(stderr, "\n");
+            }
         }
         order = nullptr;
         const uint32_t *sorted_keys = nullptr;
@@ -708,7 +734,9 @@
             seg_off[t + 1] = seg_off[t] + n_t[t];
             h_tp[t] = h_ctr[CT_TPROBES1 + t];
             h_th[t] = h_ctr[CT_THITS1 + t];
-        }
+            cx.tier_segments[t] = n_t[t];
+        }
+        cx.tier_segments[kTiers] = h_ctr[CT_TAIL_UP];
         h_split_hdr = reinterpret_cast<const unsigned long long *>(h_split);
         n_runs = split_on ? (uint32_t)h_split_hdr[0] : 0u;
         n_cuts = split_on ? (uint32_t)h_split_hdr[1] : 0u;
@@ -733,6 +761,8 @@
             }
             fprintf(stderr, "; %llu barren (no arm can reach min_duplication_length: not run), %llu of them by the positions of their hits\n",
                     (unsigned long long)n_seg - placed, (unsigned long long)h_ctr[CT_CLUSTER_BARREN]);
+            fprintf(stderr, "[asgart] tail rule: thresholds (hits) of tiers 2, 4, 5: %u %u %u; %llu segment(s) moved to the next tier that holds more\n",
+                    pp.tail_hits[1], pp.tail_hits[3], pp.tail_hits[4], (unsigned long long)h_ctr[CT_TAIL_UP]);
             if (cluster_barren) {
                 float ms_a = 0.f, ms_b = 0.f, ms_p = 0.f;
                 (void)hipEventElapsedTime(&ms_a, cx.ev[EV_BARREN], cx.ev[EV_BARREN_SMALL]);
@@ -1182,18 +1212,42 @@
             for (int t = 1; t <= kTiers; ++t) fprintf(stderr, " %d: %.2f", t, (double)tier_longest(t) * 1e-5);
             fprintf(stderr, "\n");
         }
+#ifdef ASGART_SEG_TOP
+        if (opt.debug) {
+            std::vector<unsigned long long> log(4096);
+            HIP_TRY(hipMemcpy(log.data(), w.seg_slots.as<unsigned long long>() + 4096, log.size() * 8, hipMemcpyDeviceToHost));
+            for (int stat = 2; stat <= kRunsStat; ++stat) {
+                unsigned long long *l = log.data() + (size_t)kSegTopWords * (stat & 7);
+                const size_t n_log = (size_t)std::min<unsigned long long>(l[0], kSegTopWords - 1);
+                std::sort(l + 1, l + 1 + n_log, std::greater<unsigned long long>());
+                fprintf(stderr, "[asgart] %s%d: %llu segments of %.1f ms and more; the longest (ms):", stat == kRunsStat ? "runs, as tier " : "tier ",
+                        stat == kRunsStat ? Tiers::kRunsTier : stat, l[0], (double)kSegTopMin * 1e-5);
+                for (size_t i = 0; i < std::min<size_t>(n_log, 48); ++i) fprintf(stderr, " %.2f", (double)l[1 + i] * 1e-5);
+                fprintf(stderr, "\n");
+            }
+        }
+#endif
         remember_plan_estimates();
         return 0;
     }
 
+    uint64_t plan_sig() const {
+        uint64_t sig = call_sig;
+        for (int t = 1; t <= kTiers; ++t) sig = (sig ^ tail_hits[t]) * 1099511628211ull;
+        return sig;
+    }
     void plan_estimates(double *est) const {
-        const bool known = cx.plan_known && cx.plan_sig == call_sig;
-        for (int t = 0; t <= kTiers; ++t) est[t] = known && cx.plan_est[t] > 0.0 ? cx.plan_est[t] : stat_shape(t).profile_ms;
+        const bool known = cx.plan_known && cx.plan_sig == plan_sig();
+        for (int t = 0; t <= kTiers; ++t) {
+            const TierShape &sh = stat_shape(t);
+            const double profile = tail_hits[t] && sh.tail_hits && sh.tail_profile_ms > 0.0 ? sh.tail_profile_ms : sh.profile_ms;
+            est[t] = known && cx.plan_est[t] > 0.0 ? cx.plan_est[t] : profile;
+        }
     }
     void remember_plan_estimates() {
-        if (!(cx.plan_known && cx.plan_sig == call_sig))
+        if (!(cx.plan_known && cx.plan_sig == plan_sig()))
             for (double &e : cx.plan_est) e = 0.0;
-        cx.plan_sig = call_sig;
+        cx.plan_sig = plan_sig();
         cx.plan_known = true;
         for (int t = 1; t <= kTiers; ++t) {
             if (!tier_ran[t]) continue;
@@ -1210,6 +1264,12 @@
             }
             cx.plan_est[0] = runs;
         }
+        double chip_ms = 0.0;
+        auto ran = [&](int t) { return t ? tier_ran[t] : n_runs != 0; };
+        for (int t = 0; t <= kTiers; ++t)
+            if (ran(t)) chip_ms += (double)h_ctr[CT_BUSY1 + (t ? t : kRunsStat) - 1] * 1e-5 / stat_shape(t).wg_per_cu / 256.0;
+        for (int t = 0; t <= kTiers; ++t)
+            if (ran(t) && stat_shape(t).wg_per_cu == 1) cx.plan_est[t] = std::max(cx.plan_est[t], chip_ms);
     }
 
     int32_t records() {
@@ -1832,6 +1892,31 @@
     return (int64_t)st.size();
 }
 
+int32_t asgart_tier_segments(asgart_index *idx, uint64_t *out) {
+    if (!idx || !out) {
+        set_error("bad argument");
+        return ASGART_E_ARG;
+    }
+    idx->acquire_all();
+    const SearchCtx &cx = idx->ctx[idx->last_ctx];
+    for (int i = 0; i < 8; ++i) out[i] = cx.has_last ? cx.tier_segments[i] : 0;
+    idx->release_all();
+    return 0;
+}
+
+int32_t asgart_tier_profile(double *profile_ms, uint64_t *tail_hits) {
+    if (!profile_ms || !tail_hits) {
+        set_error("bad argument");
+        return ASGART_E_ARG;
+    }
+    for (int t = 0; t <= kTiers; ++t) {
+        const TierShape &sh = TierTable<uint32_t>::shape[t][0];
+        profile_ms[t] = sh.tail_hits && sh.tail_profile_ms > 0.0 ? sh.tail_profile_ms : sh.profile_ms;
+        tail_hits[t] = TierTable<uint32_t>::shape[t][0].tail_hits;
+    }
+    return 0;
+}
+
 int32_t asgart_get_stats(asgart_index *idx, uint32_t flags, asgart_stats *out) {
     if (!idx || !out) {
         set_error("bad argument");
diff --git a/asgart_amd/csrc/pipeline_dev.hpp b/asgart_amd/csrc/pipeline_dev.hpp
--- a/asgart_amd/csrc/pipeline_dev.hpp
+++ b/asgart_amd/csrc/pipeline_dev.hpp
@@ -878,6 +878,7 @@
     uint32_t k, step, G;
     unsigned long long M;
     uint32_t dense3;
+    uint32_t tail_hits[kTiers - 1];
 };
 
 constexpr int kTierBarren = kTiers + 1;
@@ -899,7 +900,14 @@
     return (((uint32_t)tier - 1u) << 29) | low;
 }
 
-__device__ inline int place_tier(uint32_t bound, unsigned long long sum, uint32_t n_probes, const PlaceParams &pp) {
+__host__ __device__ inline int next_holding_more(const uint32_t *cap, int src, int skip = 0) {
+    int dst = src + 1;
+    while (dst < kTiers && (dst == skip || cap[dst - 1] == 0u || cap[dst - 1] <= cap[src - 1])) ++dst;
+    return dst;
+}
+
+__device__ inline int place_tier(uint32_t bound, unsigned long long sum, uint32_t n_probes, const PlaceParams &pp, bool *tail_up) {
+    *tail_up = false;
     if (bound <= pp.cap[0] && sum <= pp.sum1) return 1;
     if (pp.long3 && bound <= pp.cap[2] &&
         (n_probes >= pp.long3 || (bound > pp.cap[4] && n_probes >= pp.long3_big))) {
@@ -910,6 +918,13 @@
         if (t == 3 && pp.long3) continue;
         if (bound <= pp.cap[t - 1]) {
             if (t == 6 && pp.dense6 && bound <= pp.cap[2] && sum >= (unsigned long long)pp.dense6 * n_probes) return 3;
+            if (pp.tail_hits[t - 1] && sum >= (unsigned long long)pp.tail_hits[t - 1]) {
+                const int up = next_holding_more(pp.cap, t, 3);
+                if (up >= 4 && up <= 6) {
+                    *tail_up = true;
+                    return up;
+                }
+            }
             return t;
         }
     }
@@ -973,9 +988,11 @@
         if (g >= g_end) done = true;
         if (have && done) {
             if (rp.tstar > 64u) bound = 0xFFFFFFFFu;
-            int tier = place_tier(bound, sum, n_probes, pp);
+            bool tail_up;
+            int tier = place_tier(bound, sum, n_probes, pp, &tail_up);
             if (mx > 1 && pp.force_tier > tier) tier = min(pp.force_tier, kTiers);
             if ((by_quiet || !window_cut) && segment_is_barren(pp, n_hit, g - g0)) tier = kTierBarren;
+            if (tail_up && tier != kTierBarren) atomicAdd(&ctr[CT_TAIL_UP], 1ull);
             keys[sidx] = placement_key(tier, sum, g0);
             vals[sidx] = g0;
             if (pp.seg_info)
@@ -1075,9 +1092,11 @@
         }
         if (rp.tstar > 64u) bound = 0xFFFFFFFFu;
         if (lane == 0) {
-            int tier = place_tier(bound, sum, n_probes, pp);
+            bool tail_up;
+            int tier = place_tier(bound, sum, n_probes, pp, &tail_up);
             if (mx > 1 && pp.force_tier > tier) tier = min(pp.force_tier, kTiers);
             if ((done || !window_cut) && segment_is_barren(pp, n_hit, min(g_stop, g_end) - g0)) tier = kTierBarren;
+            if (tail_up && tier != kTierBarren) atomicAdd(&ctr[CT_TAIL_UP], 1ull);
             keys[sidx] = placement_key(tier, sum, g0);
             vals[sidx] = g0;
             if (pp.seg_info)
diff --git a/include/asgart_hip.h b/include/asgart_hip.h
--- a/include/asgart_hip.h
+++ b/include/asgart_hip.h
@@ -87,6 +87,8 @@
 
 int32_t asgart_index_set_option(asgart_index *idx, const char *name, int64_t value);
 
+int32_t asgart_index_set_tail_up(asgart_index *idx, int32_t mode, int64_t hits);
+
 int64_t asgart_index_check_sa(asgart_index *idx);
 
 int32_t asgart_index_prepare(asgart_index *idx, uint64_t probe_size);
@@ -189,6 +191,9 @@
 #define ASGART_STATS_CTX(i) (((uint32_t)(i) + 1u) << 8)
 int32_t asgart_get_stats(asgart_index *idx, uint32_t flags, asgart_stats *out);
 
+int32_t asgart_tier_segments(asgart_index *idx, uint64_t *out);
+int32_t asgart_tier_profile(double *profile_ms, uint64_t *tail_hits);
+
 const char *asgart_last_error(void);
 const char *asgart_version(void);
 
```

Measured after the change: 48260 (median of 6 runs). +10.0%, better.
